# christopherkarani/Wax

Hardware: NVIDIA H100
Metric: queries/sec cosine top-10 @ 10Mx384 fp32 (higher is better)
Workload: dtype f32

## Files before the change

wax_b200/csrc/waxvs_batch.cuh:

```cuda
#pragma once
#include <cuda.h>
#include <cuda_bf16.h>

#include "waxvs_common.cuh"
#include "waxvs_scan.cuh"

namespace waxvs {

constexpr int kBatchM = 128;
constexpr int kBatchN = 128;
constexpr int kBatchKBlock = 32;
constexpr int kBatchKBlockBf16 = 64;
constexpr int kBatchRescore = 256;
constexpr int kBatchRescoreMax = 1024;
constexpr uint32_t kBatchABytes = kBatchM * 128u;
constexpr uint32_t kBatchBBytes = kBatchN * 128u;
constexpr uint32_t kBatchStageBytes = kBatchABytes + kBatchBBytes;
constexpr int kBatchStageSlots = 8;
constexpr uint32_t kBatchScoreStride = kBatchN + 8;
constexpr uint32_t kBatchScoreBytes = kBatchM * kBatchScoreStride * 4u;
constexpr int kBatchMaxStages = 6;
constexpr uint32_t kBatchSmemOptin = 227u * 1024u;
__host__ __device__ constexpr uint32_t batch_smem_bytes(int stages, int heap, uint32_t ares_kb = 0) {
    return ares_kb * kBatchABytes + stages * (ares_kb ? kBatchBBytes : kBatchStageBytes) + kBatchScoreBytes +
// ... 863 lines not shown
        const float *vp[4];
        float d[4];
#pragma unroll
        for (uint32_t r = 0; r < 4; ++r) {
            const uint32_t i = i0 + r * nwarps;
            rows[r] = static_cast<uint32_t>(sk[i < kpp ? i : i0]);
            vp[r] = p.corpus + static_cast<size_t>(rows[r]) * p.dims;
        }
        exact_row_distance_x4<METRIC>(qv, vp, p.dims, s_a2, s_sqrt_a2, lane, d);
        if (lane == 0) {
#pragma unroll
            for (uint32_t r = 0; r < 4; ++r) {
                const uint32_t i = i0 + r * nwarps;
                if (i < kpp) ek[i] = finite_f32(d[r]) ? make_key(d[r], rows[r]) : WAXVS_KEY_NONE;
            }
        }
    }
    __syncthreads();
    block_bitonic_sort(ek, p.rescore);

    if (threadIdx.x == 0) {
        uint32_t n_exact = 0;
        while (n_exact < kpp && ek[n_exact] != WAXVS_KEY_NONE) ++n_exact;
        uint32_t ok = 1;
        float tau_star = -INFINITY, tau_star16 = -INFINITY;
        if (n_exact >= p.k && METRIC == kL2) {
            if constexpr (METRIC == kL2) {
                const float dk = from_orderable_u32(static_cast<uint32_t>(ek[p.k - 1] >> 32));
                l2_proof(s_a2, s_sqrt_a2, dk, tau, __uint_as_float(*p.max_norm_bits), p.dims, p.eps_rel, excluded_any,
                         ok, tau_star, tau_star16);
            }
        } else if (n_exact >= p.k) {
            const float dk = from_orderable_u32(static_cast<uint32_t>(ek[p.k - 1] >> 32));
            const float qn = s_sqrt_a2;
            const float scale = METRIC == kCosine ? qn : qn * __uint_as_float(*p.max_norm_bits);
            const float sk_exact = METRIC == kCosine ? (1.0f - dk) * qn : 1.0f - dk;
            const float acc_slack = static_cast<float>(p.dims) * 0x1p-23f * scale;
            const float ulp_slack = 0x1p-21f * fmaxf(1.0f, fabsf(dk)) * (METRIC == kCosine ? qn : 1.0f);
            const float eps = p.eps_rel * scale * 1.01f + acc_slack + ulp_slack + 1e-30f;
            if (excluded_any && (!(sk_exact > tau + eps) || !finite_f32(eps))) ok = 0;
            const float feps = kTf32Eps * scale * 1.01f + acc_slack + ulp_slack + 1e-30f;
            const float t = sk_exact - feps;
            tau_star = finite_f32(t) ? t - fabsf(t) * 0x1p-20f - 1e-30f : -INFINITY;
            const float feps16 = kBf16Eps * scale * 1.01f + acc_slack + ulp_slack + 1e-30f;
            const float t16 = sk_exact - feps16;
            tau_star16 = finite_f32(t16) ? t16 - fabsf(t16) * 0x1p-20f - 1e-30f : -INFINITY;
        } else if (excluded_any) {
            ok = 0;
        }
        if (METRIC != kL2 && (!(s_a2 >= 0x1p-126f) || !finite_f32(s_a2))) {
            ok = 0;
            tau_star = tau_star16 = -INFINITY;
        }
        p.ok[q] = ok;
        if (p.tau_star) { p.tau_star[q] = tau_star; p.tau_star[p.tau_stride + q] = tau_star16; }
    }
    ScanParams sp{};
    sp.out = p.out + static_cast<size_t>(q) * p.k;
    sp.frame_ids = p.frame_ids; sp.id_base = p.id_base; sp.row_offset = p.row_offset; sp.row_keys = p.row_keys;
    for (uint32_t i = threadIdx.x; i < p.k; i += blockDim.x)
        write_candidate(sp, static_cast<int>(i), i < p.rescore ? ek[i] : WAXVS_KEY_NONE);
}

struct RescoreParams {
    const float *corpus, *query;
    uint32_t dims, k, n_nominees;
    const uint64_t *nominees;
    uint32_t *aux;
    const uint32_t *max_norm_bits;
    float rho_max;
    uint64_t *block_keys;
    uint32_t *ticket;
    uint32_t *work_counter;
    wax_vs_candidate *out;
    uint32_t *ok;
    const uint64_t *frame_ids, *row_keys;
    uint64_t id_base, row_offset;
    uint32_t tail_smem_bytes;
};

template <int METRIC>
__global__ void __launch_bounds__(512, 1) shadow_rescore_kernel(const RescoreParams p) {
    static_assert(METRIC == kCosine || METRIC == kDot, "the shadow route covers cosine and dot");
    extern __shared__ __align__(16) unsigned char rsm[];
    __shared__ float s_a2, s_sqrt_a2;
    const int warp = threadIdx.x >> 5, lane = threadIdx.x & 31, warps = blockDim.x >> 5;
    const int k = static_cast<int>(p.k);
    if (warp == 0) {
        float s0 = 0.f, s1 = 0.f, s2 = 0.f, s3 = 0.f;
        for (uint32_t base = 4u * lane; base < p.dims; base += 128u) {
            const float4 x = __ldg(reinterpret_cast<const float4 *>(p.query + base));
            s0 = __fmaf_rn(x.x, x.x, s0); s1 = __fmaf_rn(x.y, x.y, s1);
            s2 = __fmaf_rn(x.z, x.z, s2); s3 = __fmaf_rn(x.w, x.w, s3);
        }
        const float a2 = warp_butterfly_sum(__fadd_rn(__fadd_rn(s0, s1), __fadd_rn(s2, s3)));
        if (lane == 0) { s_a2 = a2; s_sqrt_a2 = __fsqrt_rn(a2); }
    }
    __shared__ ScanParams sp;
    for (uint32_t i = threadIdx.x; i < sizeof(ScanParams) / 4u; i += blockDim.x) reinterpret_cast<uint32_t *>(&sp)[i] = 0u;
    __syncthreads();
    if (threadIdx.x == 0) {
        sp.k = p.k; sp.block_keys = p.block_keys; sp.ticket = p.ticket; sp.out = p.out;
        sp.frame_ids = p.frame_ids; sp.id_base = p.id_base; sp.row_offset = p.row_offset; sp.row_keys = p.row_keys;
        sp.tail_smem_bytes = p.tail_smem_bytes; sp.work_counter = p.work_counter;
    }
    __syncthreads();

    WarpTopK<1> tk;
    tk.init();
    const uint32_t stride = gridDim.x * warps * 4u;
    for (uint32_t i0 = (blockIdx.x * warps + warp) * 4u; i0 < p.n_nominees; i0 += stride) {
        uint64_t nk[4];
        const float *vp[4];
        float d[4];
#pragma unroll
        for (uint32_t r = 0; r < 4; ++r) {
            nk[r] = i0 + r < p.n_nominees ? p.nominees[i0 + r] : WAXVS_KEY_NONE;
            vp[r] = p.corpus + static_cast<size_t>(nk[r] == WAXVS_KEY_NONE ? 0u : static_cast<uint32_t>(nk[r])) * p.dims;
        }
        exact_row_distance_x4<METRIC>(p.query, vp, p.dims, s_a2, s_sqrt_a2, lane, d);
#pragma unroll
        for (uint32_t r = 0; r < 4; ++r) {
            if (nk[r] == WAXVS_KEY_NONE || !finite_f32(d[r])) continue;
            const uint64_t x = make_key(d[r], static_cast<uint32_t>(nk[r]));
            if (x < tk.thresh) tk.insert(x, lane, k);
        }
    }

    if (!finish_topk_select<1>(sp, tk, rsm)) return;
    __syncthreads();
    if (threadIdx.x != 0) return;
    const wax_vs_candidate kth = p.out[p.k - 1];
    const uint32_t cut = p.aux[0];
    const bool excluded_any = cut != WAXVS_UKEY_NONE;
    const float tau = excluded_any ? -from_orderable_u32(cut) : -INFINITY;
    const float rho_q = __uint_as_float(p.aux[1]);
    uint32_t ok = 1;
    if (kth.valid) {
        const float dk = kth.distance, qn = s_sqrt_a2;
        const float m = METRIC == kCosine ? 1.0f : __uint_as_float(*p.max_norm_bits);
        const float scale = qn * m;
        const float sk_exact = METRIC == kCosine ? (1.0f - dk) * qn : 1.0f - dk;
        const float coding = qn * p.rho_max + rho_q * ((METRIC == kCosine ? 1.0001f : m) + p.rho_max);
        const float acc_slack = static_cast<float>(p.dims) * 0x1p-23f * scale;
        const float ulp_slack = 0x1p-21f * fmaxf(1.0f, fabsf(dk)) * (METRIC == kCosine ? qn : 1.0f);
        const float eps = coding * 1.01f + acc_slack + ulp_slack + 1e-30f;
        if (excluded_any && (!(sk_exact > tau + eps) || !finite_f32(eps))) ok = 0;
    } else if (excluded_any) {
        ok = 0;
    }
    if (!(s_a2 >= 0x1p-126f) || !finite_f32(s_a2)) ok = 0;
    *p.ok = ok;
    p.aux[0] = WAXVS_UKEY_NONE;
    p.aux[2] = cut;
}

template <int METRIC>
__global__ void __launch_bounds__(256) filter_rescore_kernel(const float *corpus, const float *queries, uint32_t dims,
                                                             const uint32_t *cand_count, const uint32_t *cand_rows,
                                                             uint32_t cand_cap, uint64_t *keys) {
    const uint32_t q = blockIdx.y;
    const int lane = threadIdx.x & 31;
    const uint32_t n = min(cand_count[q], cand_cap);
    const uint32_t warps = (gridDim.x * blockDim.x) >> 5;
    uint32_t i = (blockIdx.x * blockDim.x + threadIdx.x) >> 5;
    if (i >= n) return;
// ... 64 lines not shown
```

wax_b200/csrc/waxvs_common.cuh:

```cuda
#pragma once
#include <cuda_runtime.h>
#include <stdint.h>

#define WAXVS_KEY_NONE 0xFFFFFFFFFFFFFFFFull
#define WAXVS_UKEY_NONE 0xFFFFFFFFu
#define WAXVS_FULL_MASK 0xFFFFFFFFu

namespace waxvs {

enum Metric : int { kCosine = 0, kDot = 1, kL2 = 2 };

__device__ __forceinline__ uint32_t orderable_u32(float f) {
    uint32_t u = __float_as_uint(f);
    return u ^ ((u & 0x80000000u) ? 0xFFFFFFFFu : 0x80000000u);
}
__device__ __forceinline__ float from_orderable_u32(uint32_t k) {
    uint32_t u = k ^ ((k & 0x80000000u) ? 0x80000000u : 0xFFFFFFFFu);
    return __uint_as_float(u);
}
__host__ __device__ __forceinline__ bool finite_f32(float f) {
#ifdef __CUDA_ARCH__
    return (__float_as_uint(f) & 0x7F800000u) != 0x7F800000u;
#else
    union { float f; uint32_t u; } x; x.f = f;
// ... 169 lines not shown
                if (pos < 32) {
                    if (lane == pos) key[j] = x;
                    else if (lane > pos) key[j] = up;
                    carry = last;
                    carried = true;
                }
            } else {
                key[j] = (lane == 0) ? carry : up;
                carry = last;
            }
            if (j * 32 + lane >= k) key[j] = WAXVS_KEY_NONE;
        }
        uint64_t t = WAXVS_KEY_NONE;
#pragma unroll
        for (int j = 0; j < E; ++j) {
            const uint64_t cand = shfl_u64(key[j], (k - 1) & 31);
            if (((k - 1) >> 5) == j) t = cand;
        }
        thresh = t;
    }
    __device__ __forceinline__ void merge_sorted(const uint64_t (&other)[E], int lane, int k) {
        if constexpr (E == 1) {
            bitonic_merge_lists<E>(key, thresh, other, lane, k);
        } else {
            TopKRegs<E> a, b;
#pragma unroll
            for (int j = 0; j < E; ++j) { a.key[j] = key[j]; b.key[j] = other[j]; }
            a.thresh = thresh; b.thresh = WAXVS_KEY_NONE;
            a = merge_lists_call<E>(a, b, lane, k);
#pragma unroll
            for (int j = 0; j < E; ++j) key[j] = a.key[j];
            thresh = a.thresh;
        }
    }
};

__device__ __forceinline__ uint32_t smem_u32(const void *p) {
    return static_cast<uint32_t>(__cvta_generic_to_shared(p));
}
__device__ __forceinline__ void mbar_init(uint64_t *bar, uint32_t count) {
    asm volatile("mbarrier.init.shared::cta.b64 [%0], %1;" ::"r"(smem_u32(bar)), "r"(count) : "memory");
}
__device__ __forceinline__ void mbar_fence_init() {
    asm volatile("fence.mbarrier_init.release.cluster;" ::: "memory");
}
__device__ __forceinline__ void mbar_arrive_expect_tx(uint64_t *bar, uint32_t bytes) {
    asm volatile("mbarrier.arrive.expect_tx.shared::cta.b64 _, [%0], %1;" ::"r"(smem_u32(bar)), "r"(bytes)
                 : "memory");
}
__device__ __forceinline__ void mbar_wait_parity(uint64_t *bar, uint32_t parity) {
    const uint32_t addr = smem_u32(bar);
    uint32_t done;
    do {
        asm volatile(
            "{\n\t.reg .pred p;\n\t"
            "mbarrier.try_wait.parity.shared::cta.b64 p, [%1], %2;\n\t"
            "selp.u32 %0, 1, 0, p;\n\t}"
            : "=r"(done)
            : "r"(addr), "r"(parity)
            : "memory");
    } while (!done);
}
__device__ __forceinline__ void bulk_copy_g2s(void *smem_dst, const void *gmem_src, uint32_t bytes,
                                              uint64_t *bar) {
    asm volatile(
        "cp.async.bulk.shared::cluster.global.mbarrier::complete_tx::bytes [%0], [%1], %2, [%3];" ::"r"(
            smem_u32(smem_dst)),
        "l"(gmem_src), "r"(bytes), "r"(smem_u32(bar))
        : "memory");
}
__device__ __forceinline__ void bulk_copy_g2s_hint(void *smem_dst, const void *gmem_src, uint32_t bytes,
                                                   uint64_t *bar, uint64_t policy) {
    asm volatile(
        "cp.async.bulk.shared::cluster.global.mbarrier::complete_tx::bytes.L2::cache_hint [%0], [%1], %2, "
        "[%3], %4;" ::"r"(smem_u32(smem_dst)),
        "l"(gmem_src), "r"(bytes), "r"(smem_u32(bar)), "l"(policy)
        : "memory");
}
__device__ __forceinline__ uint64_t l2_policy_evict_first() {
    uint64_t pol;
    asm volatile("createpolicy.fractional.L2::evict_first.b64 %0, 1.0;" : "=l"(pol));
    return pol;
}
__device__ __forceinline__ uint64_t ld_cg_u64(const uint64_t *p) {
    uint64_t v;
    asm volatile("ld.global.cg.u64 %0, [%1];" : "=l"(v) : "l"(p) : "memory");
    return v;
}

}
```

wax_b200/csrc/waxvs_engine.cu:

```cuda
#include <cuda_runtime.h>

#include <algorithm>
#include <atomic>
#include <cstdarg>
#include <cstdio>
#include <cstring>
#include <limits>
#include <map>
#include <mutex>
#include <new>
#include <shared_mutex>
#include <string>
#include <unordered_map>
#include <chrono>
#include <random>
#include <thread>
#include <unistd.h>
#include <cmath>
#include <vector>

#include "../../include/wax_vs_cuda.h"
#include "waxvs_common.cuh"
#include "waxvs_scan.cuh"
#include "waxvs_select.cuh"
// ... 60 lines not shown
            return fail(WAX_VS_ERR_CUDA, PINNED ? "failed to allocate pinned %s (%zu bytes): %s" : "failed to allocate %s (%zu bytes): %s",
                        what, n * sizeof(T), cudaGetErrorString(cudaGetLastError()));
        cap = n;
        return WAX_VS_OK;
    }
};
template <typename T> using DevBuf = Buf<T, false>;
template <typename T> using PinnedBuf = Buf<T, true>;

struct IdMap {
    std::vector<uint64_t> keys;
    std::vector<uint32_t> vals;
    size_t mask = 0, used = 0;
    static uint64_t mix(uint64_t x) {
        x ^= x >> 30; x *= 0xbf58476d1ce4e5b9ull; x ^= x >> 27; x *= 0x94d049bb133111ebull; x ^= x >> 31;
        return x;
    }
    void reset(size_t expect) {
        size_t cap = 64;
        while (cap < expect * 2 + 16) cap <<= 1;
        keys.assign(cap, 0);
        vals.assign(cap, 0xFFFFFFFFu);
        mask = cap - 1;
        used = 0;
    }
    void prefetch(uint64_t id) const {
        if (vals.empty()) return;
        const size_t i = mix(id) & mask;
        __builtin_prefetch(&keys[i]);
        __builtin_prefetch(&vals[i]);
    }
    uint32_t find(uint64_t id) const {
        if (vals.empty()) return 0xFFFFFFFFu;
        for (size_t i = mix(id) & mask;; i = (i + 1) & mask) {
            if (vals[i] == 0xFFFFFFFFu) return 0xFFFFFFFFu;
            if (keys[i] == id) return vals[i];
        }
    }
    void put(uint64_t id, uint32_t row) {
        if (vals.empty() || (used + 1) * 2 > keys.size()) grow();
        for (size_t i = mix(id) & mask;; i = (i + 1) & mask) {
            if (vals[i] == 0xFFFFFFFFu) { keys[i] = id; vals[i] = row; ++used; return; }
            if (keys[i] == id) { vals[i] = row; return; }
        }
    }
    void grow() {
        std::vector<uint64_t> ok; std::vector<uint32_t> ov;
        ok.swap(keys); ov.swap(vals);
        reset(std::max<size_t>(used * 2, 32));
        for (size_t i = 0; i < ov.size(); ++i) if (ov[i] != 0xFFFFFFFFu) put(ok[i], ov[i]);
    }
};

enum RouteForm : int { kRouteBf16, kRouteInt8, kRouteU4, kRouteForms };

struct Tuning {
    int variant = 0;
    int rows_per_step = 0;
    int stages = 0;
    int warps = 0;
    int grid = 0;
    int l2_hint = 0;
    int ldg_ctas_per_sm = 4;
    int chunk_steps = -1;
    int fused_k_max = 128;
    int batch_tensor = 1;
    int batch_min = 4;
    int time_overlap = 0;
    int batch_pair = 0;
    uint32_t tma_max_dims = 4096;
    int batch_large_k = 1;
    int batch_heap = 0;
    int batch_noinsert = 0;
    int batch_bf16 = 1;
    int batch_ares = 1;
    int batch_rescore = 0;
    int batch_retry = 1;
    int filter_bf16 = 1;
    int filter_cap = 8192;
    int inline_query = 1;
    int host_delivery = 1;
    int tail_select = 1;
    int shard_fused = 1;
    int batch_l2 = 0;
    int single_shadow = 0;
    uint64_t filter_bitset_bytes = 2ull << 30;
    int shadow_scan = 1;
    struct Route { uint64_t min_bytes; int rows_per_step = 0, warps = 0, stages = 0; };
    Route route[kRouteForms] = {
        {512ull << 20},
        {512ull << 20},
        {2048ull << 20},
    };
};

struct SearchCtx {
    cudaStream_t stream = nullptr;
    bool own_stream = false;
    const uint64_t *row_keys = nullptr;
    DevBuf<float> d_queries;
    DevBuf<wax_vs_candidate> d_out;
    PinnedBuf<float> h_queries;
    PinnedBuf<wax_vs_candidate> h_out;
    DevBuf<uint64_t> d_block_keys;
    DevBuf<uint32_t> d_ticket;
    DevBuf<uint32_t> d_dist_keys;
    DevBuf<SelectState> d_select;
    DevBuf<uint64_t> d_sel_keys;
    cudaEvent_t ev0 = nullptr, ev1 = nullptr;
    DevBuf<uint64_t> d_heaps;
    DevBuf<uint32_t> d_ok;
    PinnedBuf<uint32_t> h_ok;
    DevBuf<uint32_t> d_tau;
    DevBuf<__nv_bfloat16> d_queries_bf16;
    DevBuf<float> d_retry_q;
    DevBuf<wax_vs_candidate> d_retry_out;
    DevBuf<uint32_t> d_retry_ok;
    DevBuf<float> d_tau_star;
    PinnedBuf<float> h_tau_star;
    DevBuf<float> d_filter_tau;
    PinnedBuf<float> h_filter_tau;
    DevBuf<uint32_t> d_cand_count;
    DevBuf<uint32_t> d_cand_rows;
    DevBuf<uint64_t> d_cand_keys;
    DevBuf<uint32_t> d_mask;
    DevBuf<uint32_t> d_filter_rows;
    DevBuf<uint64_t> d_filter_spec;
    DevBuf<uint32_t> d_query_filter;
    DevBuf<uint32_t> d_retry_filter;
    DevBuf<uint2> d_gather_span;
    DevBuf<uint64_t> d_gather_keys;
    DevBuf<uint32_t> d_order;
    DevBuf<wax_vs_candidate> d_shard_local;
    DevBuf<unsigned long long> d_group_best;
    DevBuf<uint32_t> d_group_keys;
    DevBuf<uint2> d_group_spans;
    PinnedBuf<uint2> h_group_spans;
    DevBuf<ExpandItem> d_expand_items;
    DevBuf<uint64_t> d_expand[3];
    PinnedBuf<uint64_t> h_expand;
    DevBuf<uint64_t> d_bg_keys;
    PinnedBuf<uint64_t> h_bg_keys;
    DevBuf<uint32_t> d_bg_status;
    PinnedBuf<uint32_t> h_bg_status;
    DevBuf<CoverExpand> d_bg_expand;
    PinnedBuf<CoverExpand> h_bg_expand;
    DevBuf<ScoreItem> d_score_items;
    PinnedBuf<unsigned long long> h_flag;
    unsigned long long host_seq = 0;
    DevBuf<WhereNearItem> d_where_items;
    DevBuf<uint32_t> d_where_counts;
    DevBuf<uint64_t> d_term_ids;
    DevBuf<TermSpan> d_term_spans;
    DevBuf<TermUnit> d_term_units;
    DevBuf<uint32_t> d_term_counts;
    DevBuf<uint32_t> d_term_deny;
    DevBuf<uint32_t> d_proof_count;
    PinnedBuf<uint32_t> h_proof_count;
    uint32_t seen_failed = 0;
    bool last_u4 = false;
    DevBuf<uint32_t> d_u4_aux;
    ~SearchCtx() {
        if (ev0) cudaEventDestroy(ev0);
        if (ev1) cudaEventDestroy(ev1);
        if (own_stream && stream) cudaStreamDestroy(stream);
    }
};

struct wax_vs_engine {
    int device = 0;
    int sm_count = 132;
    size_t smem_optin = 0;
    uint32_t dims = 0;
    uint8_t similarity = 0;

    float *d_corpus = nullptr;
    uint64_t cap_rows = 0, n_rows = 0;

    bool ids_identity = true;
    uint64_t id_base = 0;
    std::vector<uint64_t> ids;
    IdMap map;
    bool map_valid = true;
    bool ids_sorted = true;
    DevBuf<uint64_t> d_ids;
    bool d_ids_dirty = true;
    std::mutex ids_mu;
    bool keys_set = false;
    std::vector<uint64_t> keys;
    DevBuf<uint64_t> d_keys;

    std::shared_mutex rw;
    std::mutex pool_mu;
    std::vector<SearchCtx *> pool;
    std::unordered_map<void *, SearchCtx *> stream_ctx;
    uint64_t pool_allocs = 0, pool_reuses = 0;
    Tuning tune;

    DevBuf<float> d_inv_norm;
    DevBuf<uint32_t> d_max_norm;
    DevBuf<float> d_half_sq;
    uint64_t norms_rows = 0;
    std::mutex norms_mu;
    struct Shadow {
        DevBuf<uint32_t> codes;
        DevBuf<float> scale;
        DevBuf<uint32_t> rho;
        uint64_t rows = 0;
        bool valid = false, unavailable = false;
        bool coarse = false;
        float rho_max = 0.0f, eps_rel = INFINITY;
        void release() { codes.release(); scale.release(); rows = 0; valid = false; }
        void invalidate(uint64_t keep_prefix, bool measured_bound) {
            rows = std::min(rows, keep_prefix);
            if (measured_bound || rows == 0) valid = false;
            if (keep_prefix == 0) coarse = false;
        }
    } shadows[kRouteForms];
    uint32_t u4_demoted = 0, u4_demote_window = 16;
    bool u4_probing = false;
    uint64_t single_route_queries[kRouteForms] = {};
    uint64_t batch_tensor_queries = 0, batch_fallback_queries = 0;
    uint64_t batch_bf16_queries = 0, batch_retry_queries = 0, batch_tf32_queries = 0, batch_filter_bf16_queries = 0;
    uint64_t filter_bitset_passes = 0;
    bool groups_set = false;
    std::vector<uint64_t> groups;
    struct GroupIndex {
        DevBuf<uint32_t> perm, row_group, starts;
        DevBuf<uint64_t> ids;
        uint32_t n_groups = 0;
        bool valid = false;
    } gindex;
    std::mutex group_mu;
    uint64_t group_index_builds = 0;
    bool attrs_set = false;
    std::vector<AttrRow> attrs;
    DevBuf<AttrRow> d_attrs;
    bool attrs_dev_valid = false;
    std::mutex attrs_mu;
    uint64_t attribute_uploads = 0;
    bool locs_set = false;
    std::vector<LocRow> locs;
    DevBuf<LocRow> d_locs;
    bool locs_dev_valid = false;
    uint64_t location_uploads = 0;
    struct TermRef {
        uint64_t off;
        uint32_t n;
    };
    bool terms_set = false;
    std::vector<TermRef> term_refs;
    std::vector<uint64_t> term_pool;
    uint64_t term_garbage = 0;
    struct TermIndex {
        DevBuf<uint64_t> keys, start;
        DevBuf<uint32_t> postings;
        DevBuf<uint64_t> sort_keys, sorted_keys;
        DevBuf<uint32_t> sort_rows, heads, numbering;
        DevBuf<uint8_t> temp;
        uint32_t n_terms = 0;
        uint64_t n_postings = 0;
        bool valid = false;
        void release_scratch() {
            sort_keys.release(); sorted_keys.release(); sort_rows.release(); heads.release(); numbering.release();
            temp.release();
        }
        void release() {
            keys.release(); start.release(); postings.release();
            release_scratch();
            n_terms = 0;
            n_postings = 0;
            valid = false;
        }
    } tindex;
    std::mutex term_mu;
    uint64_t term_index_builds = 0;
    uint64_t grouped_batch_covered_queries = 0, grouped_batch_expanded_groups = 0, grouped_batch_fallback_queries = 0;
    uint64_t grouped_batch_expansion_passes = 0;
    uint64_t shard_grouped_expanded_groups = 0;
    uint32_t bf16_skip_batches = 0;
    uint32_t shadow_scan_skip = 0;
    uint32_t heap_bump = 0, heap_bump_ttl = 0, heap_backoff = 256;
    bool heap_probing = false;
    uint32_t last_heap = 0;
    struct Ingest {
        cudaStream_t stream = nullptr;
        cudaEvent_t ev[2] = {nullptr, nullptr};
        uint8_t *pin[2] = {nullptr, nullptr};
        size_t pin_bytes = 0;
        DevBuf<float> d_stage;
        DevBuf<uint32_t> d_index;
        int threads = 1;
        ~Ingest() {
            for (int i = 0; i < 2; ++i) {
                if (pin[i]) cudaFreeHost(pin[i]);
                if (ev[i]) cudaEventDestroy(ev[i]);
            }
            if (stream) cudaStreamDestroy(stream);
        }
    } ing;
    uint64_t ingest_h2d_bytes = 0, ingest_d2h_bytes = 0;
    std::mutex ingest_mu;
    std::atomic<bool> async_pending{false};
    unsigned long long *debug_trace = nullptr;
// ... 30 lines not shown
    e->tindex.release();
    e->d_attrs.release();
    e->d_locs.release();
    if (SearchCtx *c = e->shard.ctx) {
        c->d_filter_rows.release();
        c->d_mask.release();
        c->d_term_deny.release();
    }
}

static void compact_term_pool(wax_vs_engine *e) {
    if (e->term_garbage * 2 <= e->term_pool.size()) return;
    std::vector<uint64_t> pool;
    pool.reserve(e->term_pool.size() - e->term_garbage);
    for (auto &t : e->term_refs) {
        const uint64_t off = pool.size();
        pool.insert(pool.end(), e->term_pool.begin() + t.off, e->term_pool.begin() + t.off + t.n);
        t.off = t.n ? off : 0;
    }
    e->term_pool.swap(pool);
    e->term_garbage = 0;
}
static void clear_terms(wax_vs_engine *e) {
    e->terms_set = false;
    e->term_refs.clear(); e->term_refs.shrink_to_fit();
    e->term_pool.clear(); e->term_pool.shrink_to_fit();
    e->term_garbage = 0;
    e->tindex.release();
}

static int32_t ctx_new(wax_vs_engine *e, SearchCtx **out, bool with_stream) {
    SearchCtx *c = new (std::nothrow) SearchCtx();
    if (!c) return fail(WAX_VS_ERR_CUDA, "out of host memory");
    auto bail = [&](int32_t rc) { delete c; return rc; };
    if (with_stream) {
        if (cudaStreamCreateWithFlags(&c->stream, cudaStreamNonBlocking) != cudaSuccess)
            return bail(fail(WAX_VS_ERR_CUDA, "cudaStreamCreate failed"));
        c->own_stream = true;
    }
    const size_t block_keys = static_cast<size_t>(std::max(e->sm_count * 8, 2048)) * 128;
    if (cudaMalloc(&c->d_block_keys.p, block_keys * sizeof(uint64_t)) != cudaSuccess ||
        cudaMalloc(&c->d_ticket.p, 4 * sizeof(uint32_t)) != cudaSuccess ||
        cudaMemset(c->d_ticket, 0, 4 * sizeof(uint32_t)) != cudaSuccess ||
        cudaEventCreate(&c->ev0) != cudaSuccess || cudaEventCreate(&c->ev1) != cudaSuccess)
        return bail(fail(WAX_VS_ERR_CUDA, "failed to allocate search scratch: %s",
                         cudaGetErrorString(cudaGetLastError())));
    c->d_block_keys.cap = block_keys;
    c->d_ticket.cap = 4;
    *out = c;
    return WAX_VS_OK;
}

static int32_t ctx_acquire(wax_vs_engine *e, SearchCtx **out) {
    {
        std::lock_guard<std::mutex> g(e->pool_mu);
        if (!e->pool.empty()) {
            *out = e->pool.back();
            e->pool.pop_back();
            ++e->pool_reuses;
            (*out)->row_keys = nullptr;
            return WAX_VS_OK;
        }
        ++e->pool_allocs;
    }
    return ctx_new(e, out, true);
}
static void ctx_release(wax_vs_engine *e, SearchCtx *c) {
    std::lock_guard<std::mutex> g(e->pool_mu);
    e->pool.push_back(c);
}
struct CtxLease {
    wax_vs_engine *e;
    SearchCtx *c = nullptr;
    bool clears_trace = false;
    explicit CtxLease(wax_vs_engine *eng, bool clear_trace = false) : e(eng), clears_trace(clear_trace) {}
    CtxLease(const CtxLease &) = delete;
    CtxLease &operator=(const CtxLease &) = delete;
    ~CtxLease() {
        if (c) ctx_release(e, c);
        if (clears_trace) e->debug_trace = nullptr;
    }
    int32_t acquire() { return ctx_acquire(e, &c); }
};
static int32_t ctx_for_stream(wax_vs_engine *e, void *cuda_stream, SearchCtx **out) {
    std::lock_guard<std::mutex> pg(e->pool_mu);
    auto it = e->stream_ctx.find(cuda_stream);
    if (it != e->stream_ctx.end()) {
        *out = it->second;
        (*out)->row_keys = device_row_keys(e);
        return WAX_VS_OK;
    }
    SearchCtx *c = nullptr;
    int32_t rc = ctx_new(e, &c, false);
    if (rc) return rc;
    c->stream = static_cast<cudaStream_t>(cuda_stream);
    c->row_keys = device_row_keys(e);
    e->stream_ctx[cuda_stream] = c;
    ++e->pool_allocs;
    *out = c;
    return WAX_VS_OK;
}

struct TmaConfig { int C, R, warps, stages; size_t smem; };

constexpr int kUnrolledC[7] = {1, 2, 3, 4, 6, 8, 12};
static int unrolled_index(uint32_t d) {
    for (int i = 0; i < 7; ++i)
        if (d == 128u * kUnrolledC[i]) return i;
    return -1;
}
static size_t tma_smem_budget(const wax_vs_engine *e) { return (e->smem_optin ? e->smem_optin : 232448) - 4096; }
static size_t tma_ring_smem(int warps, int stages, size_t stage_bytes) {
    return static_cast<size_t>(warps) * stages * (stage_bytes + 8 + 4) + static_cast<size_t>(warps) * 1024 + 16;
}

static bool pick_tma_config(const wax_vs_engine *e, TmaConfig *cfg, int mode = 0) {
    const uint32_t d = e->dims;
    if (d % 4u != 0) return false;
    const size_t budget = tma_smem_budget(e);
    const int ci = unrolled_index(d);
    const int C = ci < 0 ? 0 : kUnrolledC[ci];
    if (C == 0 && d < 32) return false;
    if (C == 0 && d > e->tune.tma_max_dims) return false;
    int R, warps_default = 8;
    if (C == 0) {
        int auto_r = d > 256 ? 4 : 8;
        if (d > 640) { auto_r = 8; while (auto_r > 1 && static_cast<size_t>(auto_r) * d * 4 > 32768) auto_r >>= 1; }
        if (d > 3072) auto_r = 1;
        const int want_r = e->tune.rows_per_step;
        R = (want_r == 1 || want_r == 2 || want_r == 4 || want_r == 8) ? want_r : auto_r;
        if (R == 8) warps_default = 16;
        else if (R == 4) warps_default = 12;
    } else if (C == 12) {
        R = e->tune.rows_per_step == 1 || e->tune.rows_per_step == 2 ? e->tune.rows_per_step : 2;
    } else if (C >= 6) {
        R = e->tune.rows_per_step == 2 || e->tune.rows_per_step == 4 ? e->tune.rows_per_step : 2;
    } else {
        R = e->tune.rows_per_step == 4 || e->tune.rows_per_step == 8 ? e->tune.rows_per_step : (C <= 2 ? 8 : 4);
        if (C == 1) warps_default = 16;
        else if (C == 2) warps_default = 12;
        else if (mode == 1 && static_cast<uint64_t>(e->n_rows) * d * 4 < (8ull << 30)) warps_default = 16;
    }
    const int stages = e->tune.stages > 0 ? e->tune.stages : 2;
    const size_t stage_bytes = static_cast<size_t>(R) * d * sizeof(float);
    const size_t query_bytes = C == 0 ? (static_cast<size_t>(d) * 4 + 512 + 32) : 0;
    auto smem_for = [&](int w) { return tma_ring_smem(w, stages, stage_bytes) + query_bytes; };
    int warps = std::max(1, std::min(16, e->tune.warps ? e->tune.warps : warps_default));
    if (!e->tune.warps) while (warps > 2 && smem_for(warps) > budget) --warps;
    if (smem_for(warps) > budget) return false;
    cfg->C = C; cfg->R = R; cfg->warps = warps; cfg->stages = stages; cfg->smem = smem_for(warps);
    return true;
}

template <typename K>
static cudaError_t grant_smem(wax_vs_engine *e, K kernel, size_t bytes) {
    static std::mutex mu;
    static std::map<std::pair<int, const void *>, int> granted;
    std::lock_guard<std::mutex> g(mu);
    int &have = granted[{e->device, reinterpret_cast<const void *>(kernel)}];
    if (have >= static_cast<int>(bytes)) return cudaSuccess;
    cudaError_t err = cudaFuncSetAttribute(kernel, cudaFuncAttributeMaxDynamicSharedMemorySize, static_cast<int>(bytes));
    if (err == cudaSuccess) have = static_cast<int>(bytes);
    return err;
}

template <int C, int R, int M, int E, bool EMIT, bool SHADOW = false, bool INT8 = false, bool U4 = false>
static cudaError_t launch_tma_inst(wax_vs_engine *e, const ScanParams &p, int grid, const TmaConfig &cfg, cudaStream_t s) {
    cudaError_t err = grant_smem(e, scan_tma_kernel<C, R, M, E, EMIT, SHADOW, INT8, U4>, cfg.smem);
    if (err != cudaSuccess) return err;
    scan_tma_kernel<C, R, M, E, EMIT, SHADOW, INT8, U4><<<grid, cfg.warps * 32, cfg.smem, s>>>(p);
    return cudaGetLastError();
}
template <int C, int R>
static cudaError_t launch_tma_cr(wax_vs_engine *e, const ScanParams &p, int grid, const TmaConfig &cfg, int metric, int mode,
                                 cudaStream_t s) {
    switch (metric * 3 + mode) {
        case 0: return launch_tma_inst<C, R, kCosine, 1, false>(e, p, grid, cfg, s);
        case 1: return launch_tma_inst<C, R, kCosine, 4, false>(e, p, grid, cfg, s);
        case 2: return launch_tma_inst<C, R, kCosine, 1, true>(e, p, grid, cfg, s);
        case 3: return launch_tma_inst<C, R, kDot, 1, false>(e, p, grid, cfg, s);
        case 4: return launch_tma_inst<C, R, kDot, 4, false>(e, p, grid, cfg, s);
        case 5: return launch_tma_inst<C, R, kDot, 1, true>(e, p, grid, cfg, s);
        case 6: return launch_tma_inst<C, R, kL2, 1, false>(e, p, grid, cfg, s);
        case 7: return launch_tma_inst<C, R, kL2, 4, false>(e, p, grid, cfg, s);
        default: return launch_tma_inst<C, R, kL2, 1, true>(e, p, grid, cfg, s);
    }
}
static cudaError_t launch_tma(wax_vs_engine *e, const ScanParams &p, int grid, const TmaConfig &cfg, int metric, int mode,
                              cudaStream_t s) {
#define WAXVS_CASE(Cv, Rv) if (cfg.C == Cv && cfg.R == Rv) return launch_tma_cr<Cv, Rv>(e, p, grid, cfg, metric, mode, s)
    WAXVS_CASE(1, 4); WAXVS_CASE(1, 8); WAXVS_CASE(2, 4); WAXVS_CASE(2, 8);
    WAXVS_CASE(3, 4); WAXVS_CASE(3, 8); WAXVS_CASE(4, 4); WAXVS_CASE(4, 8);
    WAXVS_CASE(6, 2); WAXVS_CASE(6, 4); WAXVS_CASE(8, 2); WAXVS_CASE(8, 4);
    WAXVS_CASE(12, 1); WAXVS_CASE(12, 2);
    WAXVS_CASE(0, 1); WAXVS_CASE(0, 2); WAXVS_CASE(0, 4); WAXVS_CASE(0, 8);
#undef WAXVS_CASE
    return cudaErrorInvalidValue;
}
template <RouteForm F, int C, int R>
static cudaError_t launch_route_cr(wax_vs_engine *e, const ScanParams &p, int grid, const TmaConfig &cfg, int metric,
                                   cudaStream_t s) {
    if constexpr (F == kRouteU4) {
        return launch_tma_inst<C, R, kDot, 4, false, true, false, true>(e, p, grid, cfg, s);
    } else {
        return metric == kCosine ? launch_tma_inst<C, R, kCosine, 4, false, true, F == kRouteInt8>(e, p, grid, cfg, s)
                                 : launch_tma_inst<C, R, kDot, 4, false, true, F == kRouteInt8>(e, p, grid, cfg, s);
    }
}
#define WAXVS_CASE(Cv, Rv) \
    if (cfg.C == Cv && cfg.R == Rv) return p ? launch_route_cr<F, Cv, Rv>(e, *p, grid, cfg, metric, s) : cudaSuccess
static cudaError_t launch_shadow_scan(wax_vs_engine *e, const ScanParams *p, int grid, const TmaConfig &cfg, int metric,
                                      cudaStream_t s) {
    constexpr RouteForm F = kRouteBf16;
    WAXVS_CASE(1, 8); WAXVS_CASE(1, 16); WAXVS_CASE(2, 8); WAXVS_CASE(2, 16);
    WAXVS_CASE(3, 4); WAXVS_CASE(3, 8); WAXVS_CASE(3, 16); WAXVS_CASE(4, 4); WAXVS_CASE(4, 8);
    WAXVS_CASE(6, 2); WAXVS_CASE(6, 4); WAXVS_CASE(8, 2); WAXVS_CASE(8, 4); WAXVS_CASE(12, 2); WAXVS_CASE(12, 4);
    return cudaErrorInvalidValue;
}
static cudaError_t launch_int8_scan(wax_vs_engine *e, const ScanParams *p, int grid, const TmaConfig &cfg, int metric,
                                   cudaStream_t s) {
    constexpr RouteForm F = kRouteInt8;
    WAXVS_CASE(1, 8); WAXVS_CASE(1, 16); WAXVS_CASE(2, 8); WAXVS_CASE(2, 16);
    WAXVS_CASE(3, 4); WAXVS_CASE(3, 8); WAXVS_CASE(3, 16); WAXVS_CASE(4, 4); WAXVS_CASE(4, 8);
    WAXVS_CASE(6, 4); WAXVS_CASE(6, 8); WAXVS_CASE(8, 4); WAXVS_CASE(12, 4);
    return cudaErrorInvalidValue;
}
static cudaError_t launch_u4_scan(wax_vs_engine *e, const ScanParams *p, int grid, const TmaConfig &cfg, int metric,
                                  cudaStream_t s) {
    constexpr RouteForm F = kRouteU4;
    WAXVS_CASE(1, 8); WAXVS_CASE(1, 16); WAXVS_CASE(2, 8); WAXVS_CASE(2, 16); WAXVS_CASE(3, 8); WAXVS_CASE(3, 16);
    WAXVS_CASE(4, 4); WAXVS_CASE(4, 8); WAXVS_CASE(6, 4); WAXVS_CASE(6, 8); WAXVS_CASE(8, 4); WAXVS_CASE(12, 4);
    return cudaErrorInvalidValue;
}
#undef WAXVS_CASE

struct RouteFormSpec {
    const char *name;
    uint32_t bits;
    bool scaled;
    cudaError_t (*launch)(wax_vs_engine *, const ScanParams *, int, const TmaConfig &, int, cudaStream_t);
    int default_r[7];
    int warps, stages;
    bool keep_warps;
    bool grid_rescore;
    uint32_t tail_bytes;
    float max_eps_rel;
};
constexpr RouteFormSpec kRouteSpec[kRouteForms] = {
    {"bf16", 16, false, launch_shadow_scan, {8, 8, 4, 4, 2, 2, 2}, 16, 3, false, false, 2, kBf16Eps},
    {"int8", 8, true, launch_int8_scan, {8, 8, 8, 4, 4, 4, 4}, 16, 3, false, false, 1, kBf16Eps},
    {"4-bit", 4, true, launch_u4_scan, {16, 16, 16, 8, 8, 4, 4}, 16, 3, true, true, 2, std::numeric_limits<float>::max()},
};
// ... 54 lines not shown
        }
    }
}

static int32_t stage_queries(wax_vs_engine *e, SearchCtx *c, const float *queries, uint32_t n, cudaStream_t stream,
                             const uint32_t *order = nullptr) {
    const size_t qfloats = static_cast<size_t>(n) * e->dims;
    int32_t rc = c->d_queries.ensure(qfloats, "query buffer");
    if (!rc) rc = c->h_queries.ensure(qfloats, "query staging");
    if (rc) return rc;
    if (order) {
        for (uint32_t j = 0; j < n; ++j)
            memcpy(c->h_queries + static_cast<size_t>(j) * e->dims, queries + static_cast<size_t>(order[j]) * e->dims,
                   e->dims * sizeof(float));
    } else {
        memcpy(c->h_queries, queries, qfloats * sizeof(float));
    }
    CUDA_TRY(cudaMemcpyAsync(c->d_queries, c->h_queries, qfloats * sizeof(float), cudaMemcpyHostToDevice, stream));
    return WAX_VS_OK;
}

struct HostDelivery {
    const float *h_query;
    wax_vs_candidate *host_out;
    unsigned long long *host_flag;
    unsigned long long seq;
    bool delivered = false;
};

static int32_t enqueue_select(wax_vs_engine *e, SearchCtx *c, const uint32_t *keys, uint32_t n, uint32_t k,
                              const ScanParams &p, cudaStream_t stream, uint64_t *launches) {
    int32_t rc = c->d_select.ensure(1, "selection state");
    if (!rc) rc = c->d_sel_keys.ensure(16384, "selected keys");
    if (rc) return rc;
    const int sgrid = std::max(1, std::min<int>(e->sm_count * 4, static_cast<int>((n + 511) / 512)));
    select_init_kernel<<<1, 256, 0, stream>>>(c->d_select, k);
    for (int pass = 0; pass < kSelectPasses; ++pass) {
        select_hist_kernel<<<sgrid, 512, 0, stream>>>(keys, n, c->d_select, pass);
        select_scan_kernel<<<1, 1024, 0, stream>>>(c->d_select, pass);
    }
    select_compact_kernel<<<sgrid, 512, 0, stream>>>(keys, n, c->d_select, c->d_sel_keys, 16384);
    uint32_t pow2 = 64;
    while (pow2 < k) pow2 <<= 1;
    CUDA_TRY(grant_smem(e, select_sort_kernel, pow2 * sizeof(uint64_t)));
    select_sort_kernel<<<1, 1024, pow2 * sizeof(uint64_t), stream>>>(c->d_select, c->d_sel_keys, pow2, p);
    CUDA_TRY(cudaGetLastError());
    *launches += 3 + 2 * kSelectPasses;
    return WAX_VS_OK;
}

static int tma_grid(const wax_vs_engine *e, const SearchCtx *c, const TmaConfig &cfg, ScanParams &p) {
    p.stages = static_cast<uint32_t>(cfg.stages);
    const uint64_t steps = (e->n_rows + cfg.R - 1) / cfg.R;
    const int max_grid = e->tune.grid > 0 ? e->tune.grid : e->sm_count;
    int grid = static_cast<int>(std::min<uint64_t>(max_grid, (steps + cfg.warps - 1) / cfg.warps));
    grid = std::max(std::min(grid, static_cast<int>(c->d_block_keys.cap / 128)), 1);
    if (e->tune.chunk_steps < 0)
        p.chunk_steps = static_cast<uint32_t>(std::max<uint64_t>(1, std::min<uint64_t>(8, steps / (static_cast<uint64_t>(grid) * cfg.warps * 2))));
    return grid;
}

static bool batch_bf16_wanted(const wax_vs_engine *e);
static int32_t ensure_shadow(wax_vs_engine *e, cudaStream_t stream);
static int32_t ensure_coded_shadow(wax_vs_engine *e, RouteForm f, cudaStream_t stream, bool keep_coarse);
static int32_t ensure_route_shadow(wax_vs_engine *e, RouteForm f, cudaStream_t stream, bool keep_coarse = false) {
    return f == kRouteBf16 ? ensure_shadow(e, stream) : ensure_coded_shadow(e, f, stream, keep_coarse);
}

constexpr uint32_t kShadowNominees = 128;
constexpr uint32_t kShadowRescore = 256;
constexpr uint32_t kShadowSkipQueries = 16;
static bool shadow_route_applies(const wax_vs_engine *e) {
    return e->tune.shadow_scan && (e->similarity == WAX_VS_COSINE || e->similarity == WAX_VS_DOT) && !e->debug_trace &&
           e->tune.batch_bf16 != 0 && e->dims % kBatchKBlockBf16 == 0 &&
           e->n_rows * e->dims * sizeof(float) >= e->tune.route[kRouteBf16].min_bytes;
}
static int32_t select_route_form(wax_vs_engine *e, cudaStream_t stream, bool demoted, bool *use, RouteForm *form,
                                 TmaConfig *cfg) {
    *use = false;
    for (const RouteForm f : {kRouteU4, kRouteInt8, kRouteBf16}) {
        if ((f == kRouteU4 && demoted) || e->n_rows * e->dims * sizeof(float) < e->tune.route[f].min_bytes ||
            !pick_route_config(e, f, cfg))
            continue;
        if (const int32_t rc = ensure_route_shadow(e, f, stream)) return rc;
        if (e->shadows[f].valid && e->shadows[f].eps_rel <= kRouteSpec[f].max_eps_rel) {
            *use = true;
            *form = f;
            return WAX_VS_OK;
        }
    }
    return WAX_VS_OK;
}

static int32_t enqueue_shadow_nominations(wax_vs_engine *e, SearchCtx *c, const ScanParams &p, const TmaConfig &cfg,
                                          cudaStream_t stream, uint64_t *launches, uint32_t *shape, RouteForm f) {
    const RouteFormSpec &fs = kRouteSpec[f];
    const wax_vs_engine::Shadow &sh = e->shadows[f];
    int32_t rc;
    if (fs.grid_rescore && !c->d_u4_aux) {
        if ((rc = c->d_u4_aux.ensure(3, "4-bit route state"))) return rc;
        CUDA_TRY(cudaMemsetAsync(c->d_u4_aux, 0xFF, 3 * sizeof(uint32_t), stream));
    }
    const size_t cta_keys = static_cast<size_t>(std::max(e->tune.grid, e->sm_count)) * kU4CtaNominees;
    if ((rc = c->d_heaps.ensure(std::max(static_cast<size_t>(kShadowNominees) * kNomineeStride, fs.grid_rescore ? cta_keys : 0), "nominee keys")) ||
        (rc = c->d_ok.ensure(1, "proof flags")) || (!p.query && (rc = c->d_queries.ensure(e->dims, "query buffer"))))
        return rc;

    ScanParams sp = p;
    sp.corpus = reinterpret_cast<const float *>(sh.codes.p);
    sp.row_scale = fs.scaled ? sh.scale.p : nullptr;
    sp.u4_aux = fs.grid_rescore ? c->d_u4_aux.p : nullptr;
    sp.k = kShadowNominees;
    sp.out = nullptr; sp.host_out = nullptr; sp.host_flag = nullptr;
    sp.nominees = c->d_heaps;
    sp.query_store = p.query ? nullptr : c->d_queries.p;
    sp.tail_select = e->tune.tail_select ? 1u : 0u;
    sp.tail_smem_bytes = static_cast<uint32_t>(static_cast<size_t>(cfg.warps) * cfg.stages * cfg.R * e->dims * fs.tail_bytes);
    const int grid = tma_grid(e, c, cfg, sp);
    CUDA_TRY(fs.launch(e, &sp, grid, cfg, e->similarity, stream));

    if (fs.grid_rescore) {
        RescoreParams rp{};
        rp.corpus = e->d_corpus; rp.query = p.query ? p.query : c->d_queries.p;
        rp.dims = e->dims; rp.k = p.k; rp.n_nominees = static_cast<uint32_t>(grid) * kU4CtaNominees;
        rp.nominees = c->d_heaps; rp.aux = c->d_u4_aux; rp.max_norm_bits = e->d_max_norm; rp.rho_max = sh.rho_max;
        rp.block_keys = c->d_block_keys; rp.ticket = c->d_ticket; rp.work_counter = sp.work_counter; rp.out = p.out; rp.ok = c->d_ok;
        rp.frame_ids = p.frame_ids; rp.id_base = p.id_base; rp.row_offset = p.row_offset; rp.row_keys = p.row_keys;
        rp.tail_smem_bytes = static_cast<uint32_t>(grid) * p.k * sizeof(uint64_t);
        if (rp.tail_smem_bytes > 48u * 1024u) rp.tail_smem_bytes = 0;
        const auto kernel = e->similarity == WAX_VS_COSINE ? shadow_rescore_kernel<kCosine> : shadow_rescore_kernel<kDot>;
        kernel<<<grid, 512, rp.tail_smem_bytes, stream>>>(rp);
        CUDA_TRY(cudaGetLastError());
    } else {
        FinishParams fp{};
        fp.corpus = e->d_corpus; fp.queries = p.query ? p.query : c->d_queries.p;
        fp.n_rows = p.n_rows; fp.dims = e->dims; fp.n_queries = 1; fp.groups = 1; fp.slices = 1;
        fp.kprime = kShadowNominees; fp.k = p.k; fp.metric = e->similarity;
        fp.heaps = c->d_heaps; fp.max_norm_bits = e->d_max_norm;
        fp.out = p.out; fp.ok = c->d_ok;
        fp.frame_ids = p.frame_ids; fp.id_base = p.id_base; fp.row_offset = p.row_offset; fp.row_keys = p.row_keys;
        fp.pow2_all = 512; fp.rescore = kShadowRescore; fp.eps_rel = sh.eps_rel;
        const size_t fsmem = static_cast<size_t>(fp.pow2_all + fp.rescore) * sizeof(uint64_t);
        const auto kernel = e->similarity == WAX_VS_COSINE ? batch_finish_kernel<kCosine> : batch_finish_kernel<kDot>;
        CUDA_TRY(grant_smem(e, kernel, fsmem));
        kernel<<<1, 512, fsmem, stream>>>(fp);
        CUDA_TRY(cudaGetLastError());
    }
    *launches += 2;
    if (shape) {
        const uint32_t s[7] = {static_cast<uint32_t>(cfg.C), static_cast<uint32_t>(cfg.R), static_cast<uint32_t>(cfg.warps),
                               static_cast<uint32_t>(cfg.stages), static_cast<uint32_t>(grid), sp.chunk_steps, sp.tail_select};
        std::copy(s, s + 7, shape);
    }
    return WAX_VS_OK;
}

static int32_t enqueue_shadow_route(wax_vs_engine *e, SearchCtx *c, ScanParams &p, cudaStream_t stream, uint64_t *launches) {
    if (!shadow_route_applies(e)) return WAX_VS_OK;
    int32_t rc;
    if (!c->h_proof_count) {
        if ((rc = c->d_proof_count.ensure(2, "proof counts")) || (rc = c->h_proof_count.ensure(2, "proof count mirror"))) return rc;
        CUDA_TRY(cudaMemsetAsync(c->d_proof_count, 0, 2 * sizeof(uint32_t), stream));
        c->h_proof_count[0] = c->h_proof_count[1] = 0;
        c->seen_failed = 0;
    }
    bool demoted;
    {
        std::lock_guard<std::mutex> pg(e->pool_mu);
        const uint32_t failed = *static_cast<volatile uint32_t *>(c->h_proof_count + 1);
        if (failed != c->seen_failed) {
            c->seen_failed = failed;
            if (c->last_u4) {
                if (e->u4_probing) e->u4_demote_window = std::min(e->u4_demote_window * 2, 1u << 20);
                e->u4_demoted = e->u4_demote_window;
            } else {
                e->shadow_scan_skip = kShadowSkipQueries;
            }
        } else if (c->last_u4 && e->u4_probing) {
            e->u4_demote_window = 16;
        }
        if (c->last_u4) e->u4_probing = false;
        c->last_u4 = false;
        if (e->shadow_scan_skip > 0) { --e->shadow_scan_skip; return WAX_VS_OK; }
        demoted = e->u4_demoted > 0;
        if (demoted && --e->u4_demoted == 0) e->u4_probing = true;
    }
    bool use = false;
    RouteForm form = kRouteBf16;
    TmaConfig cfg{};
    if ((rc = select_route_form(e, stream, demoted, &use, &form, &cfg)) || !use) return rc;
    if ((rc = enqueue_shadow_nominations(e, c, p, cfg, stream, launches, nullptr, form))) return rc;
    c->last_u4 = form == kRouteU4;
    {
        std::lock_guard<std::mutex> pg(e->pool_mu);
        ++e->single_route_queries[form];
    }
    p.proof_ok = c->d_ok;
    p.proof_count = c->d_proof_count;
    p.proof_count_host = c->h_proof_count;
    return WAX_VS_OK;
}

static ScanParams scan_params(const wax_vs_engine *e, SearchCtx *c, const float *d_query, uint32_t k_eff, uint64_t row_offset,
                              wax_vs_candidate *d_out, const uint64_t *d_ids, const uint32_t *d_mask) {
    ScanParams p{};
    p.corpus = e->d_corpus; p.query = d_query;
    p.n_rows = static_cast<uint32_t>(e->n_rows); p.dims = e->dims; p.k = k_eff;
    p.block_keys = c->d_block_keys; p.ticket = c->d_ticket; p.out = d_out;
    p.frame_ids = d_ids; p.id_base = e->id_base; p.row_offset = row_offset; p.row_keys = c->row_keys;
    p.use_l2_hint = e->tune.l2_hint ? 1u : 0u;
    p.chunk_steps = e->tune.chunk_steps > 0 ? static_cast<uint32_t>(e->tune.chunk_steps) : 0u;
    p.work_counter = c->d_ticket + 1;
    p.mask = d_mask;
    p.trace = e->debug_trace;
    return p;
}

static int32_t place_host_query(wax_vs_engine *e, SearchCtx *c, ScanParams &p, const float *h_query, bool inline_ok,
                                cudaStream_t stream) {
    if (inline_ok && e->tune.inline_query != 0 && e->dims <= static_cast<uint32_t>(kInlineQueryFloats)) {
        memcpy(p.query_inline, h_query, e->dims * sizeof(float));
        p.query = nullptr;
        return WAX_VS_OK;
    }
    int32_t rc = stage_queries(e, c, h_query, 1, stream);
    if (rc) return rc;
    p.query = c->d_queries;
    return WAX_VS_OK;
}

static int32_t enqueue_exchange(const ShardParams &sp, const wax_vs_candidate *local, uint32_t k, cudaStream_t stream,
                                uint64_t *launches) {
    shard_exchange_kernel<<<1, 256, 0, stream>>>(sp, local, k);
    CUDA_TRY(cudaGetLastError());
    ++*launches;
    return WAX_VS_OK;
}

static int32_t enqueue_search(wax_vs_engine *e, SearchCtx *c, const float *d_query, uint32_t k_eff,
                              uint64_t row_offset, wax_vs_candidate *d_out, const uint64_t *d_ids,
                              cudaStream_t stream, uint64_t *launches, const uint32_t *d_mask = nullptr,
                              const ShardParams *shard = nullptr, const HostDelivery *host = nullptr,
                              bool keys_only = false, bool shadow_route = false) {
    wax_vs_candidate *d_merged = nullptr;
    if (shard) {
        if (k_eff > static_cast<uint32_t>(kShardKCap))
            return fail(WAX_VS_ERR_UNSUPPORTED, "sharded search supports top_k <= %d (got %u)", kShardKCap, k_eff);
        int32_t rc = c->d_shard_local.ensure(kShardKCap, "shard candidates");
        if (rc) return rc;
        d_merged = d_out;
        d_out = c->d_shard_local;
    }
    auto exchange_standalone = [&]() -> int32_t {
        ShardParams sp = *shard;
        sp.final_out = d_merged;
        return enqueue_exchange(sp, d_out, k_eff, stream, launches);
    };
    if (e->n_rows == 0) {
        CUDA_TRY(cudaMemsetAsync(d_out, 0, static_cast<size_t>(k_eff) * sizeof(wax_vs_candidate), stream));
        return shard ? exchange_standalone() : WAX_VS_OK;
    }
    ScanParams p = scan_params(e, c, d_query, k_eff, row_offset, d_out, d_ids, d_mask);
    const bool emit = keys_only || k_eff > static_cast<uint32_t>(e->tune.fused_k_max);
    const int mode = emit ? 2 : (k_eff <= 32 ? 0 : 1);
    if (emit) {
        int32_t rc = c->d_dist_keys.ensure(static_cast<size_t>(e->n_rows), "distance keys");
        if (rc) return rc;
        p.dist_keys = c->d_dist_keys;
    }

    TmaConfig cfg{};
    bool use_tma = (e->tune.variant != 2) && pick_tma_config(e, &cfg, mode);
    if (e->tune.variant == 1 && !use_tma)
        return fail(WAX_VS_ERR_UNSUPPORTED, "TMA-staged kernel does not support dims=%u", e->dims);
    if (host && host->h_query) {
        int32_t rc = place_host_query(e, c, p, host->h_query, use_tma && !emit, stream);
        if (rc) return rc;
    }
    if (host && host->host_out && !emit && !shard) {
        p.host_out = host->host_out; p.host_flag = host->host_flag; p.host_seq = host->seq;
        const_cast<HostDelivery *>(host)->delivered = true;
    }
    if (use_tma && !emit && e->tune.tail_select) {
        p.tail_select = 1u;
        p.tail_smem_bytes = static_cast<uint32_t>(static_cast<size_t>(cfg.warps) * cfg.stages * cfg.R * e->dims * sizeof(float));
    }
    bool fused_exchange = false;
    if (shard && !emit) {
        const size_t list_bytes = p.tail_select ? p.tail_smem_bytes
                                                : static_cast<size_t>(use_tma ? cfg.warps : 8) * 32 * (mode == 0 ? 1 : 4) * sizeof(uint64_t);
        fused_exchange = e->tune.shard_fused != 0 && static_cast<size_t>(shard->world) * k_eff * sizeof(uint32_t) <= list_bytes;
        if (fused_exchange) { p.shard = *shard; p.shard.final_out = d_merged; }
    }
    if (shadow_route && !shard && mode == 0 && use_tma && cfg.C > 0) {
        int32_t rc = enqueue_shadow_route(e, c, p, stream, launches);
        if (rc) return rc;
    }
    int grid;
    const int grid_cap = static_cast<int>(c->d_block_keys.cap / 128);
    if (use_tma) {
        grid = tma_grid(e, c, cfg, p);
        CUDA_TRY(launch_tma(e, p, grid, cfg, e->similarity, mode, stream));
    } else {
        const int max_grid = e->tune.grid > 0 ? e->tune.grid : e->sm_count * e->tune.ldg_ctas_per_sm;
        grid = static_cast<int>(std::min<uint64_t>(max_grid, (e->n_rows + 7) / 8));
        grid = std::max(std::min(grid, grid_cap), 1);
        CUDA_TRY(launch_ldg(p, grid, e->similarity, mode, stream));
    }
    ++*launches;

    if (emit && !keys_only) {
        int32_t rc = enqueue_select(e, c, c->d_dist_keys, static_cast<uint32_t>(e->n_rows), k_eff, p, stream, launches);
        if (rc) return rc;
    }
    if (shard && !fused_exchange) return exchange_standalone();
    return WAX_VS_OK;
}

static PFN_cuTensorMapEncodeTiled_v12000 tensor_map_encoder() {
    static PFN_cuTensorMapEncodeTiled_v12000 fn = nullptr;
    static std::once_flag once;
    std::call_once(once, [] {
        void *ptr = nullptr;
        cudaDriverEntryPointQueryResult q;
        if (cudaGetDriverEntryPoint("cuTensorMapEncodeTiled", &ptr, cudaEnableDefault, &q) == cudaSuccess &&
            q == cudaDriverEntryPointSuccess)
            fn = reinterpret_cast<PFN_cuTensorMapEncodeTiled_v12000>(ptr);
    });
    return fn;
}

static int32_t make_tensor_map(CUtensorMap *map, const void *base, uint64_t rows, uint32_t dims, uint32_t box_rows,
                               bool bf16 = false) {
    auto enc = tensor_map_encoder();
    if (!enc) return fail(WAX_VS_ERR_CUDA, "cuTensorMapEncodeTiled is not available from this driver");
    const size_t esize = bf16 ? sizeof(__nv_bfloat16) : sizeof(float);
    const cuuint64_t gdim[2] = {dims, rows};
    const cuuint64_t gstride[1] = {static_cast<cuuint64_t>(dims) * esize};
    const cuuint32_t box[2] = {static_cast<cuuint32_t>(bf16 ? kBatchKBlockBf16 : kBatchKBlock), box_rows};
    const cuuint32_t estr[2] = {1, 1};
    const CUresult r = enc(map, bf16 ? CU_TENSOR_MAP_DATA_TYPE_BFLOAT16 : CU_TENSOR_MAP_DATA_TYPE_FLOAT32, 2,
                           const_cast<void *>(base), gdim, gstride, box, estr, CU_TENSOR_MAP_INTERLEAVE_NONE,
                           CU_TENSOR_MAP_SWIZZLE_128B, CU_TENSOR_MAP_L2_PROMOTION_L2_256B, CU_TENSOR_MAP_FLOAT_OOB_FILL_NONE);
    if (r != CUDA_SUCCESS) return fail(WAX_VS_ERR_CUDA, "cuTensorMapEncodeTiled failed (CUresult %d)", static_cast<int>(r));
    return WAX_VS_OK;
}

static bool batch_bf16_wanted(const wax_vs_engine *e);
static bool batch_tensor_eligible(const wax_vs_engine *e, uint32_t n_queries, uint32_t k_eff) {
    const uint32_t min_batch = (e->tune.single_shadow && batch_bf16_wanted(e)) ? 1u : static_cast<uint32_t>(std::max(e->tune.batch_min, 1));
    return e->tune.batch_tensor && n_queries >= min_batch &&
           (e->similarity == WAX_VS_COSINE || e->similarity == WAX_VS_DOT || (e->similarity == WAX_VS_L2 && e->tune.batch_l2)) &&
           e->dims % kBatchKBlock == 0 &&
           e->dims <= 8192 &&
           k_eff >= 1 && e->n_rows >= 1 &&
           (k_eff <= 128 || (k_eff <= static_cast<uint32_t>(kBatchRescoreMax) && e->tune.batch_large_k &&
                             n_queries >= static_cast<uint32_t>(std::max(e->tune.batch_min, 4)) &&
                             e->n_rows >= 64ull * k_eff));
}

static int32_t ensure_norms_locked(wax_vs_engine *e, cudaStream_t stream) {
    const bool l2 = e->similarity == WAX_VS_L2;
    if (e->norms_rows == e->n_rows && e->d_inv_norm && (!l2 || e->d_half_sq)) return WAX_VS_OK;
    if (static_cast<size_t>(e->n_rows) > e->d_inv_norm.cap || !e->d_inv_norm ||
        (l2 && (static_cast<size_t>(e->n_rows) > e->d_half_sq.cap || !e->d_half_sq))) {
        e->norms_rows = 0;
        const size_t want = static_cast<size_t>(std::max<uint64_t>(e->cap_rows, std::max<uint64_t>(e->n_rows, 1)));
        int32_t rc = e->d_inv_norm.ensure(want, "row norms");
        if (!rc && l2) rc = e->d_half_sq.ensure(want, "row half squared norms");
        if (rc) return rc;
    }
    if (!e->d_max_norm) {
        int32_t rc = e->d_max_norm.ensure(1, "max row norm");
        if (rc) return rc;
        e->norms_rows = 0;
    }
    if (e->norms_rows > e->n_rows) e->norms_rows = 0;
    if (e->norms_rows == 0) CUDA_TRY(cudaMemsetAsync(e->d_max_norm, 0, sizeof(uint32_t), stream));
// ... 717 lines not shown
        parallel_memcpy(static_cast<char *>(h_dst) + off, pin[i & 1], len, g.threads);
    }
    CUDA_TRY(cudaStreamSynchronize(g.stream));
    return WAX_VS_OK;
}

static int32_t add_batch_rows(wax_vs_engine *e, const uint64_t *frame_ids, const float *rows, uint64_t n,
                              uint32_t vector_len, const uint64_t *first_key, uint64_t *out_appended) {
    if (!e) return fail(WAX_VS_ERR_NULL, "engine is NULL");
    if (out_appended) *out_appended = 0;
    if (n == 0) return WAX_VS_OK;
    if (!frame_ids || !rows) return fail(WAX_VS_ERR_NULL, "NULL argument");
    if (vector_len != e->dims)
        return fail(WAX_VS_ERR_DIMENSION, "vector dimension mismatch: expected %u, got %u", e->dims, vector_len);
    IngestTrace tr("add_batch");
    std::unique_lock<std::shared_mutex> w(e->rw);
    if (first_key && e->n_rows > 0) {
        const uint64_t last = e->keys_set ? e->keys.back() : e->n_rows - 1;
        if (*first_key <= last)
            return fail(WAX_VS_ERR_ARGUMENT, "first key %llu is not above the last row key %llu",
                        static_cast<unsigned long long>(*first_key), static_cast<unsigned long long>(last));
    }
    DeviceGuard g(e->device);
    drain_device_path(e);
    tr.mark("lock+drain");
    int32_t rc = grow_for(e, e->n_rows + n);
    if (rc) return rc;
    if (first_key && (rc = materialize_row_keys(e))) return rc;
    tr.mark("grow");
    materialize_ids(e);
    tr.mark("ids");

    std::vector<uint32_t> target(n);
    const uint64_t n0 = e->n_rows;
    bool pure_append = true;
    bool increasing = e->ids_sorted && (e->ids.empty() || frame_ids[0] > e->ids.back());
    for (uint64_t i = 1; i < n && increasing; ++i) increasing = frame_ids[i] > frame_ids[i - 1];
    if (increasing) {
        e->ids.insert(e->ids.end(), frame_ids, frame_ids + n);
        if (e->groups_set) e->groups.insert(e->groups.end(), frame_ids, frame_ids + n);
        if (e->attrs_set) e->attrs.resize(e->attrs.size() + n, AttrRow{0, 0});
        if (e->locs_set) e->locs.resize(e->locs.size() + n, LocRow{kNoLocation, 0});
        if (e->terms_set) e->term_refs.resize(e->term_refs.size() + n, wax_vs_engine::TermRef{0, 0});
        for (uint64_t i = 0; i < n; ++i) target[i] = static_cast<uint32_t>(n0 + i);
        e->n_rows += n;
        e->map_valid = false;
    } else {
        for (uint64_t i = 0; i < n; ++i) {
            if (!e->ids_sorted && i + 8 < n) e->map.prefetch(frame_ids[i + 8]);
            uint32_t row = find_row(e, frame_ids[i]);
            if (row == 0xFFFFFFFFu) {
                row = static_cast<uint32_t>(e->n_rows);
                if (e->ids_sorted && !e->ids.empty() && frame_ids[i] < e->ids.back()) {
                    e->ids_sorted = false;
                    e->map_valid = false;
                    ensure_map(e);
                }
                e->ids.push_back(frame_ids[i]);
                if (e->groups_set) e->groups.push_back(frame_ids[i]);
                if (e->attrs_set) e->attrs.push_back(AttrRow{0, 0});
                if (e->locs_set) e->locs.push_back(LocRow{kNoLocation, 0});
                if (e->terms_set) e->term_refs.push_back(wax_vs_engine::TermRef{0, 0});
                if (!e->ids_sorted) e->map.put(frame_ids[i], row);
                else e->map_valid = false;
                ++e->n_rows;
            }
            target[i] = row;
            if (row != n0 + i) pure_append = false;
        }
    }
    e->d_ids_dirty = true;
    if (out_appended) *out_appended = e->n_rows - n0;
    if (e->keys_set) {
        const uint64_t base = first_key ? *first_key : (n0 ? e->keys.back() + 1 : 0);
        for (uint64_t r = n0; r < e->n_rows; ++r) e->keys.push_back(base + (r - n0));
        if ((rc = upload_row_keys(e, n0))) return rc;
    }
    const size_t row_bytes = static_cast<size_t>(e->dims) * sizeof(float);
    tr.mark("resolve targets");
    if (pure_append) {
        invalidate_row_caches(e, n0);
        rc = upload_bytes(e, e->d_corpus + n0 * e->dims, rows, n * row_bytes);
        tr.mark("upload");
        return rc;
    }
    invalidate_row_caches(e, 0);
    {
        std::unordered_map<uint32_t, uint64_t> last;
        last.reserve(n * 2);
        for (uint64_t i = 0; i < n; ++i) last[target[i]] = i;
        for (uint64_t i = 0; i < n; ++i) if (last[target[i]] != i) target[i] = 0xFFFFFFFFu;
    }
    auto &ig = e->ing;
    if ((rc = ingest_init(e))) return rc;
    const uint64_t slab_rows = std::max<uint64_t>(1, std::min<uint64_t>(n, (size_t(256) << 20) / row_bytes));
    if ((rc = ig.d_stage.ensure(static_cast<size_t>(slab_rows) * e->dims, "upsert staging"))) return rc;
    if ((rc = ig.d_index.ensure(static_cast<size_t>(slab_rows), "upsert targets"))) return rc;
    for (uint64_t done = 0; done < n; done += slab_rows) {
        const uint64_t m = std::min(slab_rows, n - done);
        if ((rc = upload_bytes(e, ig.d_stage, rows + done * e->dims, m * row_bytes))) return rc;
        CUDA_TRY(cudaMemcpyAsync(ig.d_index, target.data() + done, m * sizeof(uint32_t), cudaMemcpyHostToDevice, ig.stream));
        scatter_rows_kernel<<<static_cast<unsigned>(m), 128, 0, ig.stream>>>(e->d_corpus, ig.d_stage, ig.d_index, m, e->dims);
        CUDA_TRY(cudaGetLastError());
        CUDA_TRY(cudaStreamSynchronize(ig.stream));
    }
    return WAX_VS_OK;
}

int32_t wax_vs_add_batch(wax_vs_engine *e, const uint64_t *frame_ids, const float *rows, uint64_t n,
                         uint32_t vector_len) {
    return add_batch_rows(e, frame_ids, rows, n, vector_len, nullptr, nullptr);
}

int32_t wax_vs_add_batch_keyed(wax_vs_engine *e, const uint64_t *frame_ids, const float *rows, uint64_t n,
                               uint32_t vector_len, uint64_t first_key, uint64_t *out_appended) {
    return add_batch_rows(e, frame_ids, rows, n, vector_len, &first_key, out_appended);
}

int32_t wax_vs_add(wax_vs_engine *e, uint64_t frame_id, const float *vector, uint32_t vector_len) {
    return wax_vs_add_batch(e, &frame_id, vector, 1, vector_len);
}

int32_t wax_vs_contains(wax_vs_engine *e, const uint64_t *frame_ids, uint64_t n, uint8_t *out) {
    if (!e) return fail(WAX_VS_ERR_NULL, "engine is NULL");
    if (n == 0) return WAX_VS_OK;
    if (!frame_ids || !out) return fail(WAX_VS_ERR_NULL, "NULL argument");
    std::shared_lock<std::shared_mutex> r(e->rw);
    std::lock_guard<std::mutex> g(e->ids_mu);
    for (uint64_t i = 0; i < n; ++i) out[i] = row_of(e, frame_ids[i]) != 0xFFFFFFFFu;
    return WAX_VS_OK;
}

int32_t wax_vs_remove_batch(wax_vs_engine *e, const uint64_t *frame_ids, uint64_t n, uint64_t *out_removed) {
    if (!e) return fail(WAX_VS_ERR_NULL, "engine is NULL");
    if (out_removed) *out_removed = 0;
    if (n == 0) return WAX_VS_OK;
    if (!frame_ids) return fail(WAX_VS_ERR_NULL, "frame_ids is NULL");
    IngestTrace tr("remove_batch");
    std::unique_lock<std::shared_mutex> w(e->rw);
    if (e->n_rows == 0) return WAX_VS_OK;
    std::vector<uint32_t> gone;
    gone.reserve(n);
    for (uint64_t i = 0; i < n; ++i) {
        const uint32_t r = row_of(e, frame_ids[i]);
        if (r != 0xFFFFFFFFu) gone.push_back(r);
    }
    if (gone.empty()) return WAX_VS_OK;
    std::sort(gone.begin(), gone.end());
    gone.erase(std::unique(gone.begin(), gone.end()), gone.end());
    DeviceGuard g(e->device);
    drain_device_path(e);
    materialize_ids(e);
    const uint64_t old_n = e->n_rows, first = gone.front(), new_n = old_n - gone.size();
    std::vector<uint32_t> src;
    src.reserve(static_cast<size_t>(new_n - first));
    {
        size_t gi = 0;
        for (uint64_t r = first; r < old_n; ++r) {
            if (gi < gone.size() && gone[gi] == r) { ++gi; continue; }
            src.push_back(static_cast<uint32_t>(r));
        }
    }
    tr.mark("resolve rows + sources");
    int32_t rc = ingest_init(e);
    if (rc) return rc;
    auto &ig = e->ing;
    const size_t row_bytes = static_cast<size_t>(e->dims) * sizeof(float);
    const uint64_t moving = src.size();
    if (moving) {
        const uint64_t slab_rows = std::max<uint64_t>(1, std::min<uint64_t>(moving, (size_t(256) << 20) / row_bytes));
        if ((rc = ig.d_stage.ensure(static_cast<size_t>(slab_rows) * e->dims, "compaction bounce buffer"))) return rc;
        if ((rc = ig.d_index.ensure(static_cast<size_t>(slab_rows), "compaction sources"))) return rc;
        if ((rc = ingest_staging(e, slab_rows * sizeof(uint32_t)))) return rc;
        for (uint64_t done = 0; done < moving; done += slab_rows) {
            const uint64_t m = std::min(slab_rows, moving - done);
            const bool contiguous = src[done + m - 1] - src[done] == m - 1;
            float *dst = e->d_corpus + (first + done) * e->dims;
            if (contiguous) {
                CUDA_TRY(cudaMemcpyAsync(ig.d_stage, e->d_corpus + static_cast<uint64_t>(src[done]) * e->dims, m * row_bytes,
                                         cudaMemcpyDeviceToDevice, ig.stream));
            } else {
                CUDA_TRY(cudaMemcpyAsync(ig.d_index, src.data() + done, m * sizeof(uint32_t), cudaMemcpyHostToDevice, ig.stream));
                const unsigned grid = static_cast<unsigned>(std::min<uint64_t>(m, static_cast<uint64_t>(e->sm_count) * 32));
                gather_rows_kernel<<<grid, 128, 0, ig.stream>>>(ig.d_stage, e->d_corpus, ig.d_index, m, e->dims);
                CUDA_TRY(cudaGetLastError());
            }
            CUDA_TRY(cudaMemcpyAsync(dst, ig.d_stage, m * row_bytes, cudaMemcpyDeviceToDevice, ig.stream));
            CUDA_TRY(cudaStreamSynchronize(ig.stream));
        }
    }
    tr.mark("compact matrix");
    if (e->terms_set)
        for (const uint32_t r : gone) e->term_garbage += e->term_refs[r].n;
    for (uint64_t j = 0; j < moving; ++j) {
        e->ids[first + j] = e->ids[src[j]];
        if (e->groups_set) e->groups[first + j] = e->groups[src[j]];
        if (e->attrs_set) e->attrs[first + j] = e->attrs[src[j]];
        if (e->locs_set) e->locs[first + j] = e->locs[src[j]];
        if (e->terms_set) e->term_refs[first + j] = e->term_refs[src[j]];
        if (e->keys_set) e->keys[first + j] = e->keys[src[j]];
    }
    e->ids.resize(new_n);
    if (e->keys_set) e->keys.resize(new_n);
    if (e->groups_set) e->groups.resize(new_n);
    if (e->attrs_set) e->attrs.resize(new_n);
    if (e->locs_set) e->locs.resize(new_n);
    if (e->terms_set) {
        e->term_refs.resize(new_n);
        compact_term_pool(e);
    }
    e->n_rows = new_n;
    e->map_valid = false;
    e->d_ids_dirty = true;
    invalidate_row_caches(e, first);
    if ((rc = upload_row_keys(e, first))) return rc;
    tr.mark("compact ids");
    if (out_removed) *out_removed = gone.size();
    return WAX_VS_OK;
}

int32_t wax_vs_remove(wax_vs_engine *e, uint64_t frame_id) {
    return wax_vs_remove_batch(e, &frame_id, 1, nullptr);
}

static int32_t enqueue_filter_level(wax_vs_engine *e, SearchCtx *c, const float *d_queries, const float *d_tau,
                                    uint32_t n_queries, uint32_t k_eff, uint64_t row_offset, wax_vs_candidate *d_out,
                                    uint32_t *d_ok, const uint64_t *d_ids, cudaStream_t stream, uint64_t *launches,
                                    bool bf16 = false, const RowFilter &rf = RowFilter{}) {
    int32_t rc = ensure_norms(e, stream);
    if (rc) return rc;
    uint32_t cap = 64;
    while ((cap < static_cast<uint32_t>(std::max(e->tune.filter_cap, 64)) || cap < k_eff) && cap < 16384u) cap <<= 1;
    if ((rc = c->d_cand_count.ensure(static_cast<size_t>(n_queries), "filter counts"))) return rc;
    if ((rc = c->d_cand_rows.ensure(static_cast<size_t>(n_queries) * cap, "filter candidates"))) return rc;
    if ((rc = c->d_cand_keys.ensure(static_cast<size_t>(n_queries) * cap, "filter keys"))) return rc;
    CUDA_TRY(cudaMemsetAsync(c->d_cand_count, 0, static_cast<size_t>(n_queries) * sizeof(uint32_t), stream));
    auto prepare = [&](const NominateChunk &ch, BatchParams &bp) -> int32_t {
        bp.tau_fixed = d_tau + ch.q0;
        bp.cand_count = c->d_cand_count + ch.q0;
        bp.cand_rows = c->d_cand_rows + static_cast<size_t>(ch.q0) * cap;
        bp.cand_cap = cap;
        return WAX_VS_OK;
    };
    auto finish = [&](const NominateChunk &ch) -> int32_t {
        const uint32_t *count = c->d_cand_count + ch.q0;
        uint64_t *keys = c->d_cand_keys + static_cast<size_t>(ch.q0) * cap;
        const auto rescore = e->similarity == WAX_VS_COSINE ? filter_rescore_kernel<kCosine>
                             : e->similarity == WAX_VS_DOT  ? filter_rescore_kernel<kDot>
                                                            : filter_rescore_kernel<kL2>;
        rescore<<<dim3(32, ch.nq), 256, 0, stream>>>(e->d_corpus, ch.queries, e->dims, count,
                                                     c->d_cand_rows + static_cast<size_t>(ch.q0) * cap, cap, keys);
        CUDA_TRY(cudaGetLastError());
        FilterSelectParams sp{};
        sp.cand_count = count; sp.keys = keys; sp.cand_cap = cap; sp.k = k_eff;
        sp.out = d_out + static_cast<size_t>(ch.q0) * k_eff; sp.ok = d_ok + ch.q0;
        sp.frame_ids = d_ids; sp.id_base = e->id_base; sp.row_offset = row_offset; sp.row_keys = c->row_keys;
        const size_t ssmem = static_cast<size_t>(cap) * sizeof(uint64_t);
        CUDA_TRY(grant_smem(e, filter_select_kernel, ssmem));
        filter_select_kernel<<<ch.nq, 1024, ssmem, stream>>>(sp);
        CUDA_TRY(cudaGetLastError());
        *launches += 2;
        return WAX_VS_OK;
    };
    return enqueue_nominate_pass(e, c, d_queries, n_queries, bf16, true, false, false, static_cast<uint32_t>(e->sm_count),
                                 rf, stream, launches, [](uint32_t, uint32_t) { return 16u; }, prepare, finish);
}

static int32_t enqueue_scans(wax_vs_engine *e, SearchCtx *c, const float *d_queries, uint32_t n, const uint32_t *qs,
                             uint32_t k_eff, uint64_t row_offset, wax_vs_candidate *d_out, const uint64_t *d_ids,
                             cudaStream_t stream, uint64_t *launches, const RowFilter &rf, bool sync_on_error,
                             bool shadow_route = false) {
    for (uint32_t i = 0; i < n; ++i) {
        const uint32_t qi = qs ? qs[i] : i;
        const int32_t rc = enqueue_search(e, c, d_queries + static_cast<size_t>(qi) * e->dims, k_eff, row_offset,
                                          d_out + static_cast<size_t>(qi) * k_eff, d_ids, stream, launches, rf.mask(qi),
                                          nullptr, nullptr, false, shadow_route);
        if (rc) {
            if (sync_on_error) cudaStreamSynchronize(stream);
            return rc;
        }
    }
    return WAX_VS_OK;
}

static int32_t run_queries_on_device(wax_vs_engine *e, SearchCtx *c, const float *d_queries, uint32_t n_queries,
                                     uint32_t k_eff, uint64_t row_offset, wax_vs_candidate *d_out, const uint64_t *d_ids,
                                     uint64_t *launches, const RowFilter &rf = RowFilter{}) {
    int32_t rc = WAX_VS_OK;
    bool tensor_path = batch_tensor_eligible(e, n_queries, k_eff), allow_bf16 = true;
    if (tensor_path) {
        std::lock_guard<std::mutex> pg(e->pool_mu);
        if (e->bf16_skip_batches > 0) { --e->bf16_skip_batches; allow_bf16 = false; }
    }
    if (tensor_path && !allow_bf16 && n_queries < static_cast<uint32_t>(std::max(e->tune.batch_min, 1))) tensor_path = false;
    if (!tensor_path)
        return enqueue_scans(e, c, d_queries, n_queries, nullptr, k_eff, row_offset, d_out, d_ids, c->stream, launches, rf, true,
                             true);
    if ((rc = c->d_ok.ensure(static_cast<size_t>(n_queries), "proof flags"))) return rc;
    if ((rc = c->h_ok.ensure(static_cast<size_t>(n_queries), "proof flag staging"))) return rc;
    if ((rc = c->d_tau_star.ensure(static_cast<size_t>(n_queries) * 2, "filter thresholds"))) return rc;
    if ((rc = c->h_tau_star.ensure(static_cast<size_t>(n_queries) * 2, "filter threshold staging"))) return rc;
// ... 276 lines not shown
        ++*launches;
    }
    return WAX_VS_OK;
}
static int32_t stage_filter_rows(wax_vs_engine *e, SearchCtx *c, const std::vector<uint32_t> &rows, size_t reserve,
                                 int32_t mode, cudaStream_t stream, uint64_t *launches) {
    int32_t rc;
    if ((rc = c->d_filter_rows.ensure(std::max<size_t>(reserve, 1), "filter rows"))) return rc;
    if (!rows.empty())
        CUDA_TRY(cudaMemcpyAsync(c->d_filter_rows, rows.data(), rows.size() * sizeof(uint32_t), cudaMemcpyHostToDevice, stream));
    if (mode < 0) return WAX_VS_OK;
    return build_filter_bits(e, c, {0, rows.size(), 0, static_cast<uint64_t>(mode)}, 1, stream, launches);
}

struct ShardHandle {
    uint32_t magic, version;
    int32_t pid, device;
    uint64_t nonce;
    uint64_t ptr;
    int32_t rank, world;
    cudaIpcMemHandle_t ipc;
    uint8_t pad[WAX_VS_SHARD_HANDLE_BYTES - 40 - sizeof(cudaIpcMemHandle_t)];
};
static_assert(sizeof(ShardHandle) == WAX_VS_SHARD_HANDLE_BYTES, "handle blob size");
static uint64_t process_nonce() {
    static const uint64_t n = [] { std::random_device rd; return (static_cast<uint64_t>(rd()) << 32) ^ rd() ^ 0x9E3779B97F4A7C15ull; }();
    return n;
}

static void shard_teardown(wax_vs_engine *e, bool free_own) {
    auto &sh = e->shard;
    if (!sh.open) return;
    cudaDeviceSynchronize();
    for (int r = 0; r < sh.world; ++r) {
        if (r != sh.rank && sh.ipc[r] && sh.box[r]) cudaIpcCloseMemHandle(sh.box[r]);
        sh.ipc[r] = false;
        if (r != sh.rank) sh.box[r] = nullptr;
    }
    sh.connected = false;
    cudaGetLastError();
    if (!free_own) return;
    if (sh.box[sh.rank]) cudaFree(sh.box[sh.rank]);
    sh.box[sh.rank] = nullptr;
    delete sh.ctx;
    sh.ctx = nullptr;
    cudaGetLastError();
    sh.open = false;
    sh.seq = 0;
}

int32_t wax_vs_shard_open(wax_vs_engine *e, int32_t rank, int32_t world, uint64_t row_offset, uint8_t *out_handle) {
    if (!e || !out_handle) return fail(WAX_VS_ERR_NULL, "NULL argument");
    if (world < 1 || world > kShardMaxRanks || rank < 0 || rank >= world)
        return fail(WAX_VS_ERR_ARGUMENT, "rank %d of %d: world must be 1..%d", rank, world, kShardMaxRanks);
    std::unique_lock<std::shared_mutex> w(e->rw);
    DeviceGuard g(e->device);
    if (!g.ok) return g.error();
    drain_device_path(e);
    shard_teardown(e, true);
    auto &sh = e->shard;
    ShardMailbox *box = nullptr;
    CUDA_TRY(cudaMalloc(&box, sizeof(ShardMailbox)));
    int32_t rc = sh.d_final.ensure(kShardKCap, "shard result");
    if (!rc) rc = sh.h_final.ensure(kShardKCap, "shard result delivery");
    if (!rc) rc = sh.h_flag.ensure(1, "shard completion flag");
    if (rc) { cudaFree(box); return rc; }
    cudaError_t err = cudaMemset(box, 0, sizeof(ShardMailbox));
    if (err == cudaSuccess) err = cudaDeviceSynchronize();
    ShardHandle h{};
    if (err == cudaSuccess) err = cudaIpcGetMemHandle(&h.ipc, box);
    if (err != cudaSuccess) {
        cudaFree(box);
        return fail(WAX_VS_ERR_CUDA, "failed to create the shard mailbox: %s", cudaGetErrorString(err));
    }
    *sh.h_flag = 0;
    if ((rc = ctx_new(e, &sh.ctx, true))) { cudaFree(box); return rc; }
    sh.rank = rank; sh.world = world; sh.row_offset = row_offset;
    sh.box[rank] = box;
    sh.open = true; sh.connected = (world == 1);
    sh.seq = 0;
    h.magic = 0x48535857u; h.version = 1; h.pid = static_cast<int32_t>(getpid()); h.device = e->device;
    h.nonce = process_nonce(); h.ptr = reinterpret_cast<uint64_t>(box); h.rank = rank; h.world = world;
    memcpy(out_handle, &h, sizeof h);
    return WAX_VS_OK;
}

int32_t wax_vs_shard_connect(wax_vs_engine *e, const uint8_t *handles, int32_t n_handles) {
    if (!e || !handles) return fail(WAX_VS_ERR_NULL, "NULL argument");
    std::unique_lock<std::shared_mutex> w(e->rw);
    auto &sh = e->shard;
    if (!sh.open) return fail(WAX_VS_ERR_ARGUMENT, "wax_vs_shard_open has not been called");
    if (n_handles != sh.world) return fail(WAX_VS_ERR_ARGUMENT, "expected %d handles, got %d", sh.world, n_handles);
    DeviceGuard g(e->device);
    if (!g.ok) return g.error();
    for (int r = 0; r < sh.world; ++r) {
        ShardHandle h;
        memcpy(&h, handles + static_cast<size_t>(r) * sizeof h, sizeof h);
        if (h.magic != 0x48535857u || h.version != 1 || h.rank != r || h.world != sh.world)
            return fail(WAX_VS_ERR_ARGUMENT, "handle %d is not rank %d of %d", r, r, sh.world);
        if (r == sh.rank) continue;
        if (h.pid == static_cast<int32_t>(getpid()) && h.nonce == process_nonce()) {
            if (h.device != e->device) {
                int can = 0;
                CUDA_TRY(cudaDeviceCanAccessPeer(&can, e->device, h.device));
                if (!can) return fail(WAX_VS_ERR_UNSUPPORTED, "device %d cannot access device %d (no P2P path)", e->device, h.device);
                cudaError_t pe = cudaDeviceEnablePeerAccess(h.device, 0);
                if (pe != cudaSuccess && pe != cudaErrorPeerAccessAlreadyEnabled)
                    return fail(WAX_VS_ERR_CUDA, "cudaDeviceEnablePeerAccess(%d) failed: %s", h.device, cudaGetErrorString(pe));
                cudaGetLastError();
            }
            sh.box[r] = reinterpret_cast<ShardMailbox *>(h.ptr);
            sh.ipc[r] = false;
        } else {
            void *ptr = nullptr;
            cudaError_t ie = cudaIpcOpenMemHandle(&ptr, h.ipc, cudaIpcMemLazyEnablePeerAccess);
            if (ie != cudaSuccess) {
                cudaGetLastError();
                return fail(WAX_VS_ERR_UNSUPPORTED, "cudaIpcOpenMemHandle for rank %d failed: %s (no P2P/IPC path between the ranks)",
                            r, cudaGetErrorString(ie));
            }
            sh.box[r] = static_cast<ShardMailbox *>(ptr);
            sh.ipc[r] = true;
        }
    }
    sh.connected = true;
    return WAX_VS_OK;
}

int32_t wax_vs_shard_close(wax_vs_engine *e) {
    if (!e) return fail(WAX_VS_ERR_NULL, "engine is NULL");
    std::unique_lock<std::shared_mutex> w(e->rw);
    DeviceGuard g(e->device);
    shard_teardown(e, false);
    return WAX_VS_OK;
}

static ShardParams shard_params_next(wax_vs_engine *e) {
    auto &sh = e->shard;
    ShardParams sp{};
    for (int r = 0; r < sh.world; ++r) sp.box[r] = sh.box[r];
    sp.rank = static_cast<uint32_t>(sh.rank); sp.world = static_cast<uint32_t>(sh.world);
    sp.seq = ++sh.seq;
    sp.timeout_ns = sh.timeout_ns;
    return sp;
}

int32_t wax_vs_shard_search_device(wax_vs_engine *e, const float *d_query, int64_t top_k, wax_vs_candidate *d_candidates,
                                   void *cuda_stream) {
    if (!e || !d_query || !d_candidates) return fail(WAX_VS_ERR_NULL, "NULL argument");
    std::shared_lock<std::shared_mutex> r(e->rw);
    if (!e->shard.connected) return fail(WAX_VS_ERR_ARGUMENT, "the shard group is not connected (wax_vs_shard_open / _connect)");
    DeviceGuard g(e->device);
    if (!g.ok) return g.error();
    const uint32_t k_eff = clamp_topk(top_k);
    if (k_eff > static_cast<uint32_t>(kShardKCap))
        return fail(WAX_VS_ERR_UNSUPPORTED, "sharded search supports top_k <= %d (got %u)", kShardKCap, k_eff);
    SearchCtx *c = nullptr;
    int32_t rc = ctx_for_stream(e, cuda_stream, &c);
    if (rc) return rc;
    e->async_pending.store(true);
    const uint64_t *d_ids = nullptr;
    if ((rc = sync_device_ids(e, &d_ids))) return rc;
    std::lock_guard<std::mutex> sg(e->shard.mu);
    ShardParams sp = shard_params_next(e);
    uint64_t launches = 0;
    return enqueue_search(e, c, d_query, k_eff, e->shard.row_offset, d_candidates, d_ids,
                          static_cast<cudaStream_t>(cuda_stream), &launches, nullptr, &sp);
}

static int32_t shard_wait_host(wax_vs_engine *e, unsigned long long seq) {
    int32_t rc = wait_host_flag(e->shard.ctx->stream, e->shard.h_flag, seq, e->shard.timeout_ns);
    if (rc == 1)
        return fail(WAX_VS_ERR_CUDA, "shard exchange timed out: a peer rank did not deliver its candidates for query #%llu", seq);
    return rc;
}

struct Clause;
static int32_t shard_search_host(wax_vs_engine *e, const float *query, uint32_t query_len, int64_t top_k, bool filtered,
                                 const uint64_t *frame_ids, uint64_t n_ids, int32_t mode, const Clause *where,
                                 uint64_t *out_ids, float *out_scores, uint32_t out_cap, uint32_t *out_n);

int32_t wax_vs_shard_search(wax_vs_engine *e, const float *query, uint32_t query_len, int64_t top_k, uint64_t *out_ids,
                            float *out_scores, uint32_t out_cap, uint32_t *out_n) {
    if (!e || !out_n) return fail(WAX_VS_ERR_NULL, "NULL argument");
    return shard_search_host(e, query, query_len, top_k, false, nullptr, 0, 0, nullptr, out_ids, out_scores, out_cap, out_n);
}

int32_t wax_vs_debug_time_shard_search(wax_vs_engine *e, uint32_t n_queries, int64_t top_k, uint64_t seed, uint32_t warmup,
                                       uint32_t iters, float *out_ms_total, uint64_t *out_launches) {
    if (!e || !out_ms_total) return fail(WAX_VS_ERR_NULL, "NULL argument");
    if (n_queries == 0) n_queries = 1;
    std::shared_lock<std::shared_mutex> r(e->rw);
    if (!e->shard.connected) return fail(WAX_VS_ERR_ARGUMENT, "the shard group is not connected (wax_vs_shard_open / _connect)");
    DeviceGuard g(e->device);
    auto &sh = e->shard;
    std::lock_guard<std::mutex> sg(sh.mu);
    SearchCtx *c = sh.ctx;
    c->row_keys = device_row_keys(e);
    const uint32_t k_eff = clamp_topk(top_k);
    int32_t rc;
    if ((rc = c->d_queries.ensure(static_cast<size_t>(n_queries) * e->dims, "query buffer"))) return rc;
    synth_fill_kernel<<<(n_queries + 255) / 256, 256, 0, c->stream>>>(c->d_queries, n_queries, e->dims, seed, 0, 1);
    CUDA_TRY(cudaGetLastError());
    const uint64_t *d_ids = nullptr;
    if ((rc = sync_device_ids(e, &d_ids))) return rc;
    uint64_t launches = 0;
    for (uint32_t it = 0; it < warmup + iters; ++it) {
        if (it == warmup) { launches = 0; CUDA_TRY(cudaEventRecord(c->ev0, c->stream)); }
        ShardParams sp = shard_params_next(e);
        rc = enqueue_search(e, c, c->d_queries + static_cast<size_t>(it % n_queries) * e->dims, k_eff, sh.row_offset,
                            sh.d_final, d_ids, c->stream, &launches, nullptr, &sp);
        if (rc) { cudaStreamSynchronize(c->stream); return rc; }
    }
    CUDA_TRY(cudaEventRecord(c->ev1, c->stream));
    CUDA_TRY(cudaStreamSynchronize(c->stream));
    CUDA_TRY(cudaEventElapsedTime(out_ms_total, c->ev0, c->ev1));
    if (out_launches) *out_launches = launches;
    return WAX_VS_OK;
}

int32_t wax_vs_merge_candidates_device(wax_vs_engine *e, const wax_vs_candidate *d_gathered, uint32_t world,
                                       uint32_t n_queries, uint32_t k, uint32_t k_out, wax_vs_candidate *d_out,
                                       void *cuda_stream) {
    if (!e || !d_gathered || !d_out) return fail(WAX_VS_ERR_NULL, "NULL argument");
    if (world == 0 || world > 1024u || k == 0 || k_out == 0 || k_out > k)
        return fail(WAX_VS_ERR_ARGUMENT, "merge: world %u, k %u, k_out %u", world, k, k_out);
    if (n_queries == 0) return WAX_VS_OK;
    DeviceGuard g(e->device);
    if (!g.ok) return g.error();
    merge_gathered_kernel<<<n_queries, 128, 0, static_cast<cudaStream_t>(cuda_stream)>>>(d_gathered, world, n_queries, k, k_out, d_out);
    CUDA_TRY(cudaGetLastError());
    return WAX_VS_OK;
}

static int32_t ensure_locations(wax_vs_engine *e, SearchCtx *c) {
    if (e->locs_dev_valid) return WAX_VS_OK;
    const size_t n = static_cast<size_t>(e->n_rows);
    int32_t rc;
    if ((rc = e->d_locs.ensure(std::max<size_t>(n, 1), "row locations"))) return rc;
    const std::vector<LocRow> none(e->locs_set ? 0 : n, LocRow{kNoLocation, 0});
    CUDA_TRY(cudaMemcpyAsync(e->d_locs, e->locs_set ? e->locs.data() : none.data(), n * sizeof(LocRow),
                             cudaMemcpyHostToDevice, c->stream));
    CUDA_TRY(cudaStreamSynchronize(c->stream));
    e->locs_dev_valid = true;
    std::lock_guard<std::mutex> pg(e->pool_mu);
    ++e->location_uploads;
    return WAX_VS_OK;
}
static int32_t ensure_attributes(wax_vs_engine *e, SearchCtx *c, bool locations = false) {
    std::lock_guard<std::mutex> lk(e->attrs_mu);
    int32_t rc;
    if (locations && (rc = ensure_locations(e, c))) return rc;
    if (e->attrs_dev_valid) return WAX_VS_OK;
    const size_t n = static_cast<size_t>(e->n_rows);
    if ((rc = e->d_attrs.ensure(std::max<size_t>(n, 1), "row attributes"))) return rc;
    if (e->attrs_set) CUDA_TRY(cudaMemcpyAsync(e->d_attrs, e->attrs.data(), n * sizeof(AttrRow), cudaMemcpyHostToDevice, c->stream));
    else CUDA_TRY(cudaMemsetAsync(e->d_attrs, 0, n * sizeof(AttrRow), c->stream));
    CUDA_TRY(cudaStreamSynchronize(c->stream));
    e->attrs_dev_valid = true;
    std::lock_guard<std::mutex> pg(e->pool_mu);
    ++e->attribute_uploads;
    return WAX_VS_OK;
}

static int32_t ensure_term_index(wax_vs_engine *e, SearchCtx *c) {
    std::lock_guard<std::mutex> lk(e->term_mu);
    auto &ti = e->tindex;
    if (ti.valid) return WAX_VS_OK;
    uint64_t n_pairs = 0;
    if (e->terms_set)
        for (const auto &t : e->term_refs) n_pairs += t.n;
    if (n_pairs > static_cast<uint64_t>(INT32_MAX))
        return fail(WAX_VS_ERR_CAPACITY, "term index of %llu (term, row) pairs: at most %d are supported",
                    static_cast<unsigned long long>(n_pairs), INT32_MAX);
    const uint32_t P = static_cast<uint32_t>(n_pairs);
    cudaStream_t s = c->stream;
    int32_t rc;
    uint32_t n_terms = 0;
    if ((rc = ti.postings.ensure(std::max<uint32_t>(P, 1), "term postings"))) return rc;
    if (P) {
        std::vector<uint64_t> h_keys(P);
        std::vector<uint32_t> h_rows(P);
        for (uint64_t r = 0, at = 0; r < e->n_rows; ++r) {
            const auto &t = e->term_refs[r];
            for (uint32_t j = 0; j < t.n; ++j, ++at) {
                h_keys[at] = e->term_pool[t.off + j];
                h_rows[at] = static_cast<uint32_t>(r);
            }
        }
        auto &keys_in = ti.sort_keys, &keys_out = ti.sorted_keys;
        auto &rows_in = ti.sort_rows, &heads = ti.heads, &incl = ti.numbering;
        auto &temp = ti.temp;
        size_t sort_bytes = 0, scan_bytes = 0;
        CUDA_TRY(cub::DeviceRadixSort::SortPairs(nullptr, sort_bytes, keys_in.p, keys_out.p, rows_in.p, ti.postings.p,
// ... 850 lines not shown
    }
    std::vector<uint32_t> written(static_cast<size_t>((e->n_rows + 31) / 32), 0u);
    std::vector<uint64_t> list;
    uint64_t assigned = 0;
    for (uint64_t i = 0; i < n; ++i) {
        const uint32_t row = row_of(e, frame_ids[i]);
        if (row == 0xFFFFFFFFu) continue;
        list.assign(terms + term_offsets[i], terms + term_offsets[i + 1]);
        std::sort(list.begin(), list.end());
        list.erase(std::unique(list.begin(), list.end()), list.end());
        auto &ref = e->term_refs[row];
        e->term_garbage += ref.n;
        ref = wax_vs_engine::TermRef{list.empty() ? 0 : e->term_pool.size(), static_cast<uint32_t>(list.size())};
        e->term_pool.insert(e->term_pool.end(), list.begin(), list.end());
        const uint32_t wd = row >> 5, b = 1u << (row & 31u);
        if (!(written[wd] & b)) { written[wd] |= b; ++assigned; }
    }
    compact_term_pool(e);
    e->tindex.release();
    if (out_assigned) *out_assigned = assigned;
    return WAX_VS_OK;
}

static int32_t term_clauses(const wax_vs_where_near *wheres, uint32_t n_wheres, const uint32_t *query_where,
                            uint32_t n_queries, const uint64_t *where_term_offsets, const uint64_t *where_terms,
                            std::vector<Clause> &clauses, std::vector<uint32_t> &qw) {
    int32_t rc;
    if ((rc = check_term_offsets(where_term_offsets, n_wheres, where_terms, kMaxWhereTerms, "where_term_offsets"))) return rc;
    if ((rc = near_clauses(wheres, n_wheres, clauses))) return rc;
    for (uint32_t w = 0; w < n_wheres; ++w) {
        std::vector<uint64_t> &terms = clauses[w].terms;
        terms.assign(where_terms + where_term_offsets[w], where_terms + where_term_offsets[w + 1]);
        std::sort(terms.begin(), terms.end());
        terms.erase(std::unique(terms.begin(), terms.end()), terms.end());
    }
    std::vector<uint32_t> canon(n_wheres);
    std::unordered_map<std::string, uint32_t> first_of;
    for (uint32_t w = 0; w < n_wheres; ++w) {
        const Clause &cl = clauses[w];
        canon[w] = w;
        if (cl.terms.empty()) continue;
        std::string key(reinterpret_cast<const char *>(&cl.pred), sizeof(WherePred));
        key.append(reinterpret_cast<const char *>(&cl.box), sizeof(LocBox));
        key.append(reinterpret_cast<const char *>(cl.terms.data()), cl.terms.size() * sizeof(uint64_t));
        canon[w] = first_of.emplace(std::move(key), w).first->second;
    }
    qw.resize(n_queries);
    for (uint32_t i = 0; i < n_queries; ++i) qw[i] = query_where[i] == WAX_VS_NO_FILTER ? WAX_VS_NO_FILTER : canon[query_where[i]];
    return WAX_VS_OK;
}

int32_t wax_vs_search_batch_where_terms(wax_vs_engine *e, const float *queries, uint32_t n_queries, uint32_t query_len,
                                        int64_t top_k, const uint64_t *frame_ids, const uint64_t *filter_offsets,
                                        const int32_t *filter_modes, uint32_t n_filters, const uint32_t *query_filter,
                                        const wax_vs_where_near *wheres, uint32_t n_wheres, const uint32_t *query_where,
                                        const uint64_t *where_term_offsets, const uint64_t *where_terms,
                                        uint64_t *out_ids, float *out_scores, uint32_t out_stride, uint32_t *out_n) {
    int32_t rc;
    if ((rc = check_where_args(e, n_queries, frame_ids, filter_offsets, filter_modes, n_filters, query_filter, wheres,
                               n_wheres, query_where, out_n)))
        return rc;
    if (!where_term_offsets) return fail(WAX_VS_ERR_NULL, "where_term_offsets is NULL");
    std::vector<Clause> clauses;
    std::vector<uint32_t> qw;
    if ((rc = term_clauses(wheres, n_wheres, query_where, n_queries, where_term_offsets, where_terms, clauses, qw)))
        return rc;
    return search_where_host(e, queries, n_queries, query_len, top_k, frame_ids, filter_offsets, filter_modes, n_filters,
                             query_filter, clauses, qw.data(), out_ids, out_scores, out_stride, out_n);
}

static int32_t reserve_shard_scratch(wax_vs_engine *e, SearchCtx *c) {
    const size_t rows = std::max<size_t>(e->n_rows, 1), words = (rows + 31) / 32;
    int32_t rc;
    if ((rc = c->d_queries.ensure(e->dims, "query buffer")) || (rc = c->h_queries.ensure(e->dims, "query staging")) ||
        (rc = c->d_out.ensure(kShardKCap, "result buffer")) || (rc = c->d_shard_local.ensure(kShardKCap, "shard candidates")) ||
        (rc = c->d_filter_rows.ensure(rows, "filter rows")) || (rc = c->d_mask.ensure(words, "row filters")) ||
        (rc = c->d_filter_spec.ensure(4, "filter spec")) || (rc = c->d_query_filter.ensure(1, "query filters")) ||
        (rc = c->d_gather_span.ensure(1, "gather spans")) || (rc = c->d_gather_keys.ensure(kWhereGatherRows, "gather keys")) ||
        (rc = c->d_where_items.ensure(1, "where predicates")) || (rc = c->d_where_counts.ensure(1, "where counts")) ||
        (rc = c->d_term_ids.ensure(kMaxWhereTerms, "required terms")) ||
        (rc = c->d_term_spans.ensure(kMaxWhereTerms, "term spans")) || (rc = c->d_term_units.ensure(1, "term units")) ||
        (rc = c->d_term_counts.ensure(1, "term counts")) || (rc = c->d_term_deny.ensure(rows, "term deny-lists")))
        return rc;
    return WAX_VS_OK;
}

static int32_t shard_search_host(wax_vs_engine *e, const float *query, uint32_t query_len, int64_t top_k, bool filtered,
                                 const uint64_t *frame_ids, uint64_t n_ids, int32_t mode, const Clause *where,
                                 uint64_t *out_ids, float *out_scores, uint32_t out_cap, uint32_t *out_n) {
    std::shared_lock<std::shared_mutex> r(e->rw);
    *out_n = 0;
    if (!e->shard.connected) return fail(WAX_VS_ERR_ARGUMENT, "the shard group is not connected (wax_vs_shard_open / _connect)");
    int32_t rc;
    if ((rc = check_query(e, query, query_len))) return rc;
    const uint32_t k_eff = clamp_topk(top_k);
    if (k_eff > static_cast<uint32_t>(kShardKCap))
        return fail(WAX_VS_ERR_UNSUPPORTED, "sharded search supports top_k <= %d (got %u)", kShardKCap, k_eff);
    if (!out_ids || !out_scores) return fail(WAX_VS_ERR_NULL, "output buffer is NULL");
    DeviceGuard g(e->device);
    if (!g.ok) return g.error();
    auto &sh = e->shard;
    std::lock_guard<std::mutex> sg(sh.mu);
    SearchCtx *c = sh.ctx;
    c->row_keys = device_row_keys(e);
    const uint64_t *d_ids = nullptr;
    if ((rc = sync_device_ids(e, &d_ids))) return rc;
    uint64_t launches = 0;
    const bool planned = filtered || where;
    const std::vector<Clause> wheres(where ? 1 : 0, where ? *where : Clause{});
    const uint32_t qw = where ? 0u : WAX_VS_NO_FILTER, qf = filtered && (mode == 0 || n_ids) ? 0u : WAX_VS_NO_FILTER;
    const uint64_t offsets[2] = {0, n_ids};
    FilterSet ids, fs;
    std::vector<int32_t> modes;
    std::vector<uint32_t> pair_of;
    FilteredPlan plan;
    if (planned && e->n_rows) {
        resolve_filters(e, frame_ids, offsets, 1, &qf, 1, ids);
        if ((rc = reserve_shard_scratch(e, c)) ||
            (rc = plan_where_pairs(e, c, wheres, &qw, &mode, &qf, 1, ids, fs, modes, pair_of)))
            return rc;
        plan_filtered(e, k_eff, modes.data(), pair_of.data(), 1, fs, plan);
    }
    ShardParams sp = shard_params_next(e);
    sp.host_out = sh.h_final; sp.host_flag = sh.h_flag;
    if (!planned) {
        HostDelivery hd{query, nullptr, nullptr, 0};
        rc = enqueue_search(e, c, nullptr, k_eff, sh.row_offset, sh.d_final, d_ids, c->stream, &launches, nullptr, &sp, &hd);
    } else if (plan.order.empty()) {
        sp.final_out = sh.d_final;
        if ((rc = c->d_shard_local.ensure(kShardKCap, "shard candidates"))) return rc;
        CUDA_TRY(cudaMemsetAsync(c->d_shard_local, 0, k_eff * sizeof(wax_vs_candidate), c->stream));
        rc = enqueue_exchange(sp, c->d_shard_local, k_eff, c->stream, &launches);
    } else {
        sp.final_out = sh.d_final;
        plan.k_max = plan.k_of[0] = k_eff;
        FilteredTarget tgt;
        tgt.row_offset = sh.row_offset; tgt.d_ids = d_ids; tgt.shard = &sp;
        rc = run_filtered(e, c, query, modes.data(), static_cast<uint32_t>(modes.size()), pair_of.data(), fs, plan, tgt);
    }
    if (rc) { cudaStreamSynchronize(c->stream); return rc; }
    if ((rc = shard_wait_host(e, sp.seq))) { cudaStreamSynchronize(c->stream); return rc; }
    if (planned) CUDA_TRY(cudaStreamSynchronize(c->stream));
    uint32_t m = 0;
    for (uint32_t i = 0; i < k_eff; ++i) {
        const wax_vs_candidate &cd = sh.h_final[i];
        if (cd.valid != 1u) continue;
        if (m >= out_cap) return fail(WAX_VS_ERR_BUFFER, "output buffers hold %u entries, need more", out_cap);
        out_ids[m] = cd.frame_id;
        out_scores[m] = score_from_distance(e->similarity, cd.distance);
        ++m;
    }
    *out_n = m;
    return WAX_VS_OK;
}

int32_t wax_vs_shard_search_where(wax_vs_engine *e, const float *query, uint32_t query_len, int64_t top_k,
                                  const uint64_t *frame_ids, uint64_t n_ids, int32_t mode, const wax_vs_where_near *where,
                                  const uint64_t *terms, uint32_t n_terms, uint64_t *out_ids, float *out_scores,
                                  uint32_t out_cap, uint32_t *out_n) {
    if (!e || !out_n || !where) return fail(WAX_VS_ERR_NULL, "NULL argument");
    if (mode != 0 && mode != 1) return fail(WAX_VS_ERR_ARGUMENT, "filter mode must be 0 (allow-list) or 1 (deny-list)");
    if (n_ids && !frame_ids) return fail(WAX_VS_ERR_NULL, "frame_ids is NULL");
    const uint64_t term_offsets[2] = {0, n_terms};
    std::vector<Clause> clauses;
    std::vector<uint32_t> qw;
    const uint32_t q0 = 0;
    int32_t rc;
    if ((rc = term_clauses(where, 1, &q0, 1, term_offsets, terms, clauses, qw))) return rc;
    return shard_search_host(e, query, query_len, top_k, true, frame_ids, n_ids, mode, &clauses[0], out_ids, out_scores,
                             out_cap, out_n);
}

int32_t wax_vs_search_batch_where_device(wax_vs_engine *e, const float *d_queries, uint32_t n_queries, int64_t top_k,
                                         const uint64_t *frame_ids, const uint64_t *filter_offsets,
                                         const int32_t *filter_modes, uint32_t n_filters, const uint32_t *query_filter,
                                         const wax_vs_where_near *wheres, uint32_t n_wheres, const uint32_t *query_where,
                                         const uint64_t *where_term_offsets, const uint64_t *where_terms,
                                         uint64_t row_offset, wax_vs_candidate *d_candidates, void *cuda_stream) {
    int32_t rc;
    uint32_t no_out_n = 0;
    if ((rc = check_where_args(e, n_queries, frame_ids, filter_offsets, filter_modes, n_filters, query_filter, wheres,
                               n_wheres, query_where, &no_out_n)))
        return rc;
    if (!d_queries || !d_candidates) return fail(WAX_VS_ERR_NULL, "NULL argument");
    std::vector<Clause> clauses;
    std::vector<uint32_t> qw;
    if (where_term_offsets) {
        rc = term_clauses(wheres, n_wheres, query_where, n_queries, where_term_offsets, where_terms, clauses, qw);
    } else {
        rc = near_clauses(wheres, n_wheres, clauses);
        qw.assign(query_where, query_where + n_queries);
    }
    if (rc) return rc;
    if (n_queries == 0) return WAX_VS_OK;
    std::shared_lock<std::shared_mutex> r(e->rw);
    DeviceGuard g(e->device);
    if (!g.ok) return g.error();
    SearchCtx *c = nullptr;
    if ((rc = ctx_for_stream(e, cuda_stream, &c))) return rc;
    const uint32_t k_out = clamp_topk(top_k);
    e->async_pending.store(true);
    CUDA_TRY(cudaMemsetAsync(d_candidates, 0, static_cast<size_t>(n_queries) * k_out * sizeof(wax_vs_candidate), c->stream));
    if (e->n_rows == 0) return WAX_VS_OK;
    const uint64_t *d_ids = nullptr;
    if ((rc = sync_device_ids(e, &d_ids))) return rc;
    FilterSet ids, fs;
    resolve_filters(e, frame_ids, filter_offsets, n_filters, query_filter, n_queries, ids);
    std::vector<int32_t> modes;
    std::vector<uint32_t> pair_of;
    if ((rc = plan_where_pairs(e, c, clauses, qw.data(), filter_modes, query_filter, n_queries, ids, fs, modes, pair_of)))
// ... 827 lines not shown
    const uint8_t magic[4] = {0x4D, 0x56, 0x32, 0x56};
    memcpy(p, magic, 4); p += 4;
    const uint16_t version = 1; memcpy(p, &version, 2); p += 2;
    *p++ = 2;
    *p++ = e->similarity;
    memcpy(p, &e->dims, 4); p += 4;
    memcpy(p, &e->n_rows, 8); p += 8;
    const uint64_t vbytes = e->n_rows * e->dims * 4ull;
    memcpy(p, &vbytes, 8); p += 8;
    memset(p, 0, 8); p += 8;
    if (vbytes) {
        std::lock_guard<std::mutex> ig(e->ingest_mu);
        int32_t rc = download_bytes(e, p, e->d_corpus, vbytes);
        if (rc) return rc;
    }
    p += vbytes;
    const uint64_t ibytes = e->n_rows * 8ull;
    memcpy(p, &ibytes, 8); p += 8;
    if (e->ids_identity) {
        for (uint64_t i = 0; i < e->n_rows; ++i) { const uint64_t id = e->id_base + i; memcpy(p + i * 8, &id, 8); }
    } else if (ibytes) {
        memcpy(p, e->ids.data(), ibytes);
    }
    return WAX_VS_OK;
}

static int32_t deserialize_rows(wax_vs_engine *e, const uint8_t *src, uint64_t len, bool all, uint64_t first, uint64_t n) {
    if (!e || !src) return fail(WAX_VS_ERR_NULL, "NULL argument");
    std::unique_lock<std::shared_mutex> w(e->rw);
    if (len < 36) return fail(WAX_VS_ERR_FORMAT, "Metal segment too small: %llu bytes", static_cast<unsigned long long>(len));
    const uint8_t magic[4] = {0x4D, 0x56, 0x32, 0x56};
    if (memcmp(src, magic, 4) != 0) return fail(WAX_VS_ERR_FORMAT, "Metal segment magic mismatch");
    uint16_t version; memcpy(&version, src + 4, 2);
    if (version != 1) return fail(WAX_VS_ERR_FORMAT, "Unsupported Metal segment version %u", version);
    if (src[6] != 2) return fail(WAX_VS_ERR_FORMAT, "Unsupported Metal segment encoding %u", src[6]);
    if (src[7] > 2 || src[7] != e->similarity)
        return fail(WAX_VS_ERR_FORMAT, "Metric mismatch: expected %u, got %u", e->similarity, src[7]);
    uint32_t dims; memcpy(&dims, src + 8, 4);
    if (dims != e->dims) return fail(WAX_VS_ERR_FORMAT, "Dimension mismatch: expected %u, got %u", e->dims, dims);
    uint64_t count, vbytes; memcpy(&count, src + 12, 8); memcpy(&vbytes, src + 20, 8);
    for (int i = 0; i < 8; ++i)
        if (src[28 + i] != 0) return fail(WAX_VS_ERR_FORMAT, "Metal segment reserved bytes must be zero");
    if (count > 0xFFFFFFFFull) return fail(WAX_VS_ERR_CAPACITY, "capacity exceeded: limit %llu, requested %llu", 0xFFFFFFFFull, static_cast<unsigned long long>(count));
    if (vbytes != count * static_cast<uint64_t>(dims) * 4ull) return fail(WAX_VS_ERR_FORMAT, "Vector data length mismatch");
    if (len < 36 + vbytes + 8) return fail(WAX_VS_ERR_FORMAT, "Metal segment missing frameId length");
    uint64_t ibytes; memcpy(&ibytes, src + 36 + vbytes, 8);
    if (ibytes != count * 8ull) return fail(WAX_VS_ERR_FORMAT, "FrameId data length mismatch");
    if (len != 36 + vbytes + 8 + ibytes)
        return fail(WAX_VS_ERR_FORMAT, "vec segment length mismatch: expected %llu, got %llu",
                    static_cast<unsigned long long>(36 + vbytes + 8 + ibytes), static_cast<unsigned long long>(len));
    if (all) first = 0, n = count;
    else if (first > count || n > count - first)
        return fail(WAX_VS_ERR_ARGUMENT, "rows [%llu, %llu + %llu) are outside the segment's %llu rows",
                    static_cast<unsigned long long>(first), static_cast<unsigned long long>(first),
                    static_cast<unsigned long long>(n), static_cast<unsigned long long>(count));
    const size_t row_bytes = static_cast<size_t>(dims) * 4u;
    DeviceGuard g(e->device);
    drain_device_path(e);
    int32_t rc = set_capacity(e, std::max<uint64_t>(n, 64));
    if (rc) return rc;
    if (n && (rc = upload_bytes(e, e->d_corpus, src + 36 + first * row_bytes, n * row_bytes)))
        return rc;
    e->n_rows = n;
    e->ids.resize(n);
    if (n) memcpy(e->ids.data(), src + 36 + vbytes + 8 + first * 8, n * 8);
    e->ids_identity = false;
    e->map_valid = false;
    e->ids_sorted = true;
    for (uint64_t i = 1; i < n && e->ids_sorted; ++i) e->ids_sorted = e->ids[i] > e->ids[i - 1];
    e->d_ids_dirty = true;
    e->keys_set = !all;
    e->keys.resize(e->keys_set ? n : 0);
    for (uint64_t i = 0; i < e->keys.size(); ++i) e->keys[i] = first + i;
    e->keys.shrink_to_fit();
    if ((rc = upload_row_keys(e, 0))) return rc;
    e->groups_set = false;
    e->groups.clear(); e->groups.shrink_to_fit();
    e->attrs_set = false;
    e->attrs.clear(); e->attrs.shrink_to_fit();
    e->locs_set = false;
    e->locs.clear(); e->locs.shrink_to_fit();
    clear_terms(e);
    invalidate_row_caches(e, 0);
    return WAX_VS_OK;
}

int32_t wax_vs_deserialize(wax_vs_engine *e, const uint8_t *src, uint64_t len) {
    return deserialize_rows(e, src, len, true, 0, 0);
}

int32_t wax_vs_deserialize_rows(wax_vs_engine *e, const uint8_t *src, uint64_t len, uint64_t first, uint64_t n) {
    return deserialize_rows(e, src, len, false, first, n);
}

int32_t wax_vs_export_rows(wax_vs_engine *e, uint64_t first, uint64_t n, uint64_t *out_ids, float *out_vectors,
                           uint64_t *out_keys) {
    if (!e) return fail(WAX_VS_ERR_NULL, "engine is NULL");
    std::shared_lock<std::shared_mutex> r(e->rw);
    if (first > e->n_rows || n > e->n_rows - first) return fail(WAX_VS_ERR_ARGUMENT, "row range out of bounds");
    for (uint64_t i = 0; i < n; ++i) {
        if (out_ids) out_ids[i] = frame_id_of(e, first + i);
        if (out_keys) out_keys[i] = e->keys_set ? e->keys[first + i] : first + i;
    }
    if (out_vectors && n) {
        DeviceGuard g(e->device);
        if (!g.ok) return g.error();
        std::lock_guard<std::mutex> ig(e->ingest_mu);
        return download_bytes(e, out_vectors, e->d_corpus + first * e->dims, n * e->dims * sizeof(float));
    }
    return WAX_VS_OK;
}

int32_t wax_vs_debug_pool_stats(wax_vs_engine *e, uint64_t *allocations, uint64_t *reuses) {
    if (!e) return fail(WAX_VS_ERR_NULL, "engine is NULL");
    std::lock_guard<std::mutex> g(e->pool_mu);
    if (allocations) *allocations = e->pool_allocs;
    if (reuses) *reuses = e->pool_reuses;
    return WAX_VS_OK;
}

int32_t wax_vs_debug_fill_synthetic(wax_vs_engine *e, uint64_t seed, uint64_t first_row, uint64_t rows,
                                    uint64_t id_base, int32_t normalize) {
    if (!e) return fail(WAX_VS_ERR_NULL, "engine is NULL");
    if (rows > 0xFFFFFFFFull) return fail(WAX_VS_ERR_CAPACITY, "capacity exceeded: limit %llu, requested %llu", 0xFFFFFFFFull, static_cast<unsigned long long>(rows));
    std::unique_lock<std::shared_mutex> w(e->rw);
    DeviceGuard g(e->device);
    drain_device_path(e);
    e->n_rows = 0;
    int32_t rc = set_capacity(e, std::max<uint64_t>(rows, 64));
    if (rc) return rc;
    if (rows) {
        const unsigned blocks = static_cast<unsigned>((rows + 255) / 256);
        synth_fill_kernel<<<blocks, 256>>>(e->d_corpus, rows, e->dims, seed, first_row, normalize);
        CUDA_TRY(cudaGetLastError());
        CUDA_TRY(cudaDeviceSynchronize());
    }
    e->n_rows = rows;
    e->ids.clear(); e->ids.shrink_to_fit();
    e->ids_identity = true; e->id_base = id_base;
    e->map = IdMap(); e->map_valid = true; e->ids_sorted = true;
    e->d_ids_dirty = true;
    e->keys_set = false;
    e->keys.clear(); e->keys.shrink_to_fit();
    e->groups_set = false;
    e->groups.clear(); e->groups.shrink_to_fit();
    e->attrs_set = false;
    e->attrs.clear(); e->attrs.shrink_to_fit();
    e->locs_set = false;
    e->locs.clear(); e->locs.shrink_to_fit();
    clear_terms(e);
    invalidate_row_caches(e, 0);
    return WAX_VS_OK;
}

int32_t wax_vs_debug_read_rows(wax_vs_engine *e, uint64_t first, uint64_t n, float *dst) {
    if (!e || !dst) return fail(WAX_VS_ERR_NULL, "NULL argument");
    std::shared_lock<std::shared_mutex> r(e->rw);
    if (first + n > e->n_rows) return fail(WAX_VS_ERR_ARGUMENT, "row range out of bounds");
    DeviceGuard g(e->device);
    if (n) CUDA_TRY(cudaMemcpy(dst, e->d_corpus + first * e->dims, n * e->dims * sizeof(float), cudaMemcpyDeviceToHost));
    return WAX_VS_OK;
}

int32_t wax_vs_debug_time_search(wax_vs_engine *e, uint32_t n_queries, int64_t top_k, uint64_t seed,
                                 uint32_t warmup, uint32_t iters, float *out_ms_total, uint64_t *out_launches) {
    if (!e || !out_ms_total) return fail(WAX_VS_ERR_NULL, "NULL argument");
    if (n_queries == 0) n_queries = 1;
    std::shared_lock<std::shared_mutex> r(e->rw);
    DeviceGuard g(e->device);
    CtxLease lease(e);
    int32_t rc = lease.acquire();
    if (rc) return rc;
    SearchCtx *c = lease.c;
    const uint32_t k_eff = clamp_topk(top_k);
    const size_t qfloats = static_cast<size_t>(n_queries) * e->dims;
    if ((rc = c->d_queries.ensure(qfloats, "query buffer"))) return rc;
    if ((rc = c->d_out.ensure(static_cast<size_t>(n_queries) * k_eff, "result buffer"))) return rc;
    synth_fill_kernel<<<(n_queries + 255) / 256, 256, 0, c->stream>>>(c->d_queries, n_queries, e->dims, seed, 0, 1);
    CUDA_TRY(cudaGetLastError());
    uint64_t launches = 0;
    CtxLease lease2(e);
    if (e->tune.time_overlap) {
        if ((rc = lease2.acquire())) return rc;
        if ((rc = lease2.c->d_out.ensure(static_cast<size_t>(n_queries) * k_eff, "result buffer"))) return rc;
    }
    SearchCtx *c2 = lease2.c;
    if (shadow_route_applies(e)) {
        bool use = false;
        RouteForm form = kRouteBf16;
        TmaConfig cfg{};
        if ((rc = select_route_form(e, c->stream, false, &use, &form, &cfg))) return rc;
    }
    for (uint32_t it = 0; it < warmup + iters; ++it) {
        if (it == warmup) {
            launches = 0;
            if (c2) { CUDA_TRY(cudaEventRecord(c2->ev0, c2->stream)); CUDA_TRY(cudaStreamWaitEvent(c->stream, c2->ev0, 0)); }
            CUDA_TRY(cudaEventRecord(c->ev0, c->stream));
            if (c2) CUDA_TRY(cudaStreamWaitEvent(c2->stream, c->ev0, 0));
        }
        const uint32_t qi = it % n_queries;
        SearchCtx *cc = (c2 && (it & 1u)) ? c2 : c;
        if (c2 && it == 0) { CUDA_TRY(cudaEventRecord(c->ev1, c->stream)); CUDA_TRY(cudaStreamWaitEvent(c2->stream, c->ev1, 0)); }
        rc = enqueue_search(e, cc, c->d_queries + static_cast<size_t>(qi) * e->dims, k_eff, 0,
                            cc->d_out + static_cast<size_t>(qi) * k_eff, nullptr, cc->stream, &launches, nullptr, nullptr,
                            nullptr, false, true);
        if (rc) { cudaStreamSynchronize(c->stream); if (c2) cudaStreamSynchronize(c2->stream); return rc; }
    }
    if (c2) { CUDA_TRY(cudaEventRecord(c2->ev1, c2->stream)); CUDA_TRY(cudaStreamWaitEvent(c->stream, c2->ev1, 0)); }
    CUDA_TRY(cudaEventRecord(c->ev1, c->stream));
    CUDA_TRY(cudaStreamSynchronize(c->stream));
    CUDA_TRY(cudaEventElapsedTime(out_ms_total, c->ev0, c->ev1));
    if (out_launches) *out_launches = launches;
    return WAX_VS_OK;
}

int32_t wax_vs_debug_stream_read(wax_vs_engine *e, uint32_t iters, float *out_best_ms, uint64_t *out_bytes) {
    if (!e || !out_best_ms || !out_bytes) return fail(WAX_VS_ERR_NULL, "NULL argument");
    std::shared_lock<std::shared_mutex> r(e->rw);
    DeviceGuard g(e->device);
    CtxLease lease(e);
    int32_t rc = lease.acquire();
    if (rc) return rc;
    SearchCtx *c = lease.c;
    const uint64_t bytes = e->n_rows * e->dims * sizeof(float) / 16 * 16;
    *out_bytes = bytes;
    *out_best_ms = 0.0f;
    if (bytes == 0) return WAX_VS_OK;
    float best = 1e30f;
    for (uint32_t it = 0; it < iters + 2; ++it) {
        CUDA_TRY(cudaEventRecord(c->ev0, c->stream));
        stream_read_kernel<<<e->sm_count * 4, 512, 0, c->stream>>>(reinterpret_cast<const uint4 *>(e->d_corpus),
                                                                     bytes / 16, c->d_ticket + 2);
        CUDA_TRY(cudaGetLastError());
        CUDA_TRY(cudaEventRecord(c->ev1, c->stream));
        CUDA_TRY(cudaStreamSynchronize(c->stream));
// ... 41 lines not shown
    if (!e || !out5) return fail(WAX_VS_ERR_NULL, "NULL argument");
    std::unique_lock<std::shared_mutex> w(e->rw);
    DeviceGuard g(e->device);
    CtxLease lease(e, true);
    int32_t rc = lease.acquire();
    if (rc) return rc;
    SearchCtx *c = lease.c;
    const uint32_t k_eff = clamp_topk(top_k);
    if ((rc = c->d_queries.ensure(static_cast<size_t>(e->dims), "query buffer"))) return rc;
    if ((rc = c->d_out.ensure(static_cast<size_t>(k_eff), "result buffer"))) return rc;
    synth_fill_kernel<<<1, 256, 0, c->stream>>>(c->d_queries, 1, e->dims, 99, 0, 1);
    unsigned long long *d_trace = nullptr;
    CUDA_TRY(cudaMalloc(&d_trace, 8 * sizeof(unsigned long long)));
    double acc[5] = {0, 0, 0, 0, 0};
    uint64_t launches = 0;
    for (uint32_t it = 0; it < iters + 3; ++it) {
        const unsigned long long init[8] = {~0ull, 0, 0, 0, 0, 0, 0, 0};
        cudaMemcpyAsync(d_trace, init, sizeof init, cudaMemcpyHostToDevice, c->stream);
        cudaStreamSynchronize(c->stream);
        e->debug_trace = d_trace;
        cudaEventRecord(c->ev0, c->stream);
        rc = enqueue_search(e, c, c->d_queries, k_eff, 0, c->d_out, nullptr, c->stream, &launches);
        cudaEventRecord(c->ev1, c->stream);
        e->debug_trace = nullptr;
        if (rc) { cudaStreamSynchronize(c->stream); cudaFree(d_trace); return rc; }
        unsigned long long t[8];
        cudaMemcpyAsync(t, d_trace, sizeof t, cudaMemcpyDeviceToHost, c->stream);
        cudaStreamSynchronize(c->stream);
        float ms = 0;
        cudaEventElapsedTime(&ms, c->ev0, c->ev1);
        if (it < 3) continue;
        for (int i = 0; i < 4; ++i) acc[i] += (t[i + 1] > t[0] && t[0] != ~0ull) ? (t[i + 1] - t[0]) * 1e-3 : 0.0;
        acc[4] += ms * 1e3;
    }
    cudaFree(d_trace);
    for (int i = 0; i < 5; ++i) out5[i] = static_cast<float>(acc[i] / std::max(iters, 1u));
    CUDA_TRY(cudaGetLastError());
    return WAX_VS_OK;
}

int32_t wax_vs_debug_batch_stats(wax_vs_engine *e, uint64_t *tensor_queries, uint64_t *fallback_queries) {
    if (!e) return fail(WAX_VS_ERR_NULL, "engine is NULL");
    std::lock_guard<std::mutex> g(e->pool_mu);
    if (tensor_queries) *tensor_queries = e->batch_tensor_queries;
    if (fallback_queries) *fallback_queries = e->batch_fallback_queries;
    return WAX_VS_OK;
}

int32_t wax_vs_debug_counter(wax_vs_engine *e, const char *name, uint64_t *out) {
    if (!e || !name || !out) return fail(WAX_VS_ERR_NULL, "NULL argument");
    std::lock_guard<std::mutex> g(e->pool_mu);
    const wax_vs_engine::Shadow &bf = e->shadows[kRouteBf16], &i8 = e->shadows[kRouteInt8], &u4 = e->shadows[kRouteU4];
    if (!strcmp(name, "batch_tensor_queries")) *out = e->batch_tensor_queries;
    else if (!strcmp(name, "batch_fallback_queries")) *out = e->batch_fallback_queries;
    else if (!strcmp(name, "batch_bf16_queries")) *out = e->batch_bf16_queries;
    else if (!strcmp(name, "batch_retry_queries")) *out = e->batch_retry_queries;
    else if (!strcmp(name, "batch_filter_bf16_queries")) *out = e->batch_filter_bf16_queries;
    else if (!strcmp(name, "shadow_bytes")) *out = bf.valid ? bf.rows * e->dims * sizeof(__nv_bfloat16) : 0;
    else if (!strcmp(name, "shadow_capacity_bytes")) *out = bf.codes.cap * sizeof(uint32_t);
    else if (!strcmp(name, "shadow_unavailable")) *out = bf.unavailable ? 1 : 0;
    else if (!strcmp(name, "batch_tf32_queries")) *out = e->batch_tf32_queries;
    else if (!strcmp(name, "filter_bitset_passes")) *out = e->filter_bitset_passes;
    else if (!strcmp(name, "group_index_builds")) *out = e->group_index_builds;
    else if (!strcmp(name, "attribute_uploads")) *out = e->attribute_uploads;
    else if (!strcmp(name, "location_uploads")) *out = e->location_uploads;
    else if (!strcmp(name, "term_index_builds")) *out = e->term_index_builds;
    else if (!strcmp(name, "term_index_bytes"))
        *out = e->tindex.keys.cap * sizeof(uint64_t) + e->tindex.start.cap * sizeof(uint64_t) + e->tindex.postings.cap * sizeof(uint32_t);
    else if (!strcmp(name, "grouped_batch_covered_queries")) *out = e->grouped_batch_covered_queries;
    else if (!strcmp(name, "grouped_batch_expanded_groups")) *out = e->grouped_batch_expanded_groups;
    else if (!strcmp(name, "grouped_batch_fallback_queries")) *out = e->grouped_batch_fallback_queries;
    else if (!strcmp(name, "grouped_batch_expansion_passes")) *out = e->grouped_batch_expansion_passes;
    else if (!strcmp(name, "shard_grouped_expanded_groups")) *out = e->shard_grouped_expanded_groups;
    else if (!strcmp(name, "ingest_h2d_bytes")) *out = e->ingest_h2d_bytes;
    else if (!strcmp(name, "ingest_d2h_bytes")) *out = e->ingest_d2h_bytes;
    else if (!strcmp(name, "norms_rows")) *out = e->norms_rows;
    else if (!strcmp(name, "shadow_rows")) *out = bf.rows;
    else if (!strcmp(name, "int8_shadow_bytes")) *out = i8.valid ? i8.rows * (e->dims + sizeof(float)) : 0;
    else if (!strcmp(name, "int8_shadow_rows")) *out = i8.rows;
    else if (!strcmp(name, "u4_shadow_bytes")) *out = u4.valid ? u4.rows * (e->dims / 2 + sizeof(float)) : 0;
    else if (!strcmp(name, "u4_shadow_rows")) *out = u4.rows;
    else if (!strcmp(name, "single_u4_queries")) *out = e->single_route_queries[kRouteU4];
    else if (!strcmp(name, "single_int8_queries")) *out = e->single_route_queries[kRouteInt8];
    else if (!strcmp(name, "batch_heap_bump")) *out = e->heap_bump;
    else if (!strcmp(name, "batch_last_heap")) *out = e->last_heap;
    else if (!strcmp(name, "single_shadow_queries") || !strcmp(name, "single_shadow_fallbacks")) {
        const int slot = !strcmp(name, "single_shadow_queries") ? 0 : 1;
        uint64_t n = 0;
        auto add = [&](const SearchCtx *c) { if (c->h_proof_count) n += *static_cast<volatile uint32_t *>(c->h_proof_count + slot); };
        for (const SearchCtx *c : e->pool) add(c);
        for (const auto &kv : e->stream_ctx) add(kv.second);
        *out = n;
    }
    else if (!strcmp(name, "pool_allocs")) *out = e->pool_allocs;
    else if (!strcmp(name, "pool_reuses")) *out = e->pool_reuses;
    else return fail(WAX_VS_ERR_ARGUMENT, "unknown counter '%s'", name);
    return WAX_VS_OK;
}

int32_t wax_vs_debug_time_search_batch(wax_vs_engine *e, uint32_t n_queries, int64_t top_k, uint64_t seed,
                                       uint32_t warmup, uint32_t iters, float *out_ms_total,
                                       uint64_t *out_launches, uint32_t *out_unproven) {
    if (!e || !out_ms_total) return fail(WAX_VS_ERR_NULL, "NULL argument");
    if (n_queries == 0) n_queries = 1;
    std::shared_lock<std::shared_mutex> r(e->rw);
    DeviceGuard g(e->device);
    const uint32_t k_eff = static_cast<uint32_t>(std::min<uint64_t>(clamp_topk(top_k), std::max<uint64_t>(e->n_rows, 1)));
    if (!batch_tensor_eligible(e, n_queries, k_eff))
        return fail(WAX_VS_ERR_UNSUPPORTED, "batch of %u queries, k=%u, dims=%u is not eligible for the tensor path", n_queries, k_eff, e->dims);
    CtxLease lease(e);
    int32_t rc = lease.acquire();
    if (rc) return rc;
    SearchCtx *c = lease.c;
    const size_t qfloats = static_cast<size_t>(n_queries) * e->dims;
    if ((rc = c->d_queries.ensure(qfloats, "query buffer"))) return rc;
    if ((rc = c->d_out.ensure(static_cast<size_t>(n_queries) * k_eff, "result buffer"))) return rc;
    if ((rc = c->d_ok.ensure(static_cast<size_t>(n_queries), "proof flags"))) return rc;
    if ((rc = c->h_ok.ensure(static_cast<size_t>(n_queries), "proof flag staging"))) return rc;
    synth_fill_kernel<<<(n_queries + 255) / 256, 256, 0, c->stream>>>(c->d_queries, n_queries, e->dims, seed, 0, 1);
    CUDA_TRY(cudaGetLastError());
    if ((rc = ensure_norms(e, c->stream))) return rc;
    if (batch_bf16_wanted(e) && (rc = ensure_shadow(e, c->stream))) return rc;
    uint64_t launches = 0;
    for (uint32_t it = 0; it < warmup + iters; ++it) {
        if (it == warmup) { launches = 0; CUDA_TRY(cudaEventRecord(c->ev0, c->stream)); }
        uint32_t used_heap = 0;
        rc = enqueue_batch_tensor(e, c, c->d_queries, n_queries, k_eff, 0, c->d_out, c->d_ok, nullptr, c->stream, &launches,
                                  true, nullptr, nullptr, RowFilter{}, &used_heap);
        if (rc) { cudaStreamSynchronize(c->stream); return rc; }
        if (used_heap) { std::lock_guard<std::mutex> pg(e->pool_mu); e->last_heap = used_heap; }
    }
    CUDA_TRY(cudaEventRecord(c->ev1, c->stream));
    CUDA_TRY(cudaMemcpyAsync(c->h_ok, c->d_ok, n_queries * sizeof(uint32_t), cudaMemcpyDeviceToHost, c->stream));
    CUDA_TRY(cudaStreamSynchronize(c->stream));
    CUDA_TRY(cudaEventElapsedTime(out_ms_total, c->ev0, c->ev1));
    if (out_launches) *out_launches = launches;
    if (out_unproven) {
        uint32_t bad = 0;
        for (uint32_t i = 0; i < n_queries; ++i) bad += c->h_ok[i] ? 0u : 1u;
        *out_unproven = bad;
    }
    return WAX_VS_OK;
}

int32_t wax_vs_debug_batch_nominations(wax_vs_engine *e, const float *queries, uint32_t n_queries, int64_t top_k,
                                       const uint32_t *allow_bits, float *out_scores, uint32_t *out_ok,
                                       uint64_t *out_heaps, uint64_t heaps_cap, uint32_t *out_shape) {
    if (!e || !queries || !out_scores || !out_ok || !out_shape) return fail(WAX_VS_ERR_NULL, "NULL argument");
    std::shared_lock<std::shared_mutex> r(e->rw);
    DeviceGuard g(e->device);
    if (!g.ok) return g.error();
    const uint32_t k_eff = static_cast<uint32_t>(std::min<uint64_t>(clamp_topk(top_k), std::max<uint64_t>(e->n_rows, 1)));
    if (n_queries == 0 || e->n_rows == 0 || k_eff > 128u || e->dims % kBatchKBlock != 0 || e->dims > 8192 ||
        (e->similarity != WAX_VS_COSINE && e->similarity != WAX_VS_DOT && !(e->similarity == WAX_VS_L2 && e->tune.batch_l2)))
        return fail(WAX_VS_ERR_UNSUPPORTED, "batch of %u queries, k=%u, dims=%u has no tensor-core nomination pass",
                    n_queries, k_eff, e->dims);
    CtxLease lease(e);
    int32_t rc = lease.acquire();
    if (rc) return rc;
    SearchCtx *c = lease.c;
    const size_t qfloats = static_cast<size_t>(n_queries) * e->dims;
    const size_t n_scores = static_cast<size_t>(n_queries) * e->n_rows;
    if ((rc = c->d_queries.ensure(qfloats, "query buffer"))) return rc;
    if ((rc = c->d_out.ensure(static_cast<size_t>(n_queries) * k_eff, "result buffer"))) return rc;
    if ((rc = c->d_ok.ensure(static_cast<size_t>(n_queries), "proof flags"))) return rc;
    DevBuf<float> scores;
    if ((rc = scores.ensure(n_scores, "nomination scores"))) return rc;
    CUDA_TRY(cudaMemsetAsync(scores, 0xFF, n_scores * sizeof(float), c->stream));
    CUDA_TRY(cudaMemcpyAsync(c->d_queries, queries, qfloats * sizeof(float), cudaMemcpyHostToDevice, c->stream));
    const uint32_t *d_mask = nullptr;
    if (allow_bits) {
        const size_t words = static_cast<size_t>((e->n_rows + 31) / 32);
        if ((rc = c->d_mask.ensure(words, "row filter"))) return rc;
        CUDA_TRY(cudaMemcpyAsync(c->d_mask, allow_bits, words * sizeof(uint32_t), cudaMemcpyHostToDevice, c->stream));
// ... 94 lines not shown
                                    uint32_t *out_shape, float *out_bound) {
    return debug_route_nominations(e, query, top_k, allow_bits, out_keys, out_ok, out_result, out_shape, kRouteU4,
                                   keys_cap, out_bound);
}

static int32_t debug_read_route_shadow(wax_vs_engine *e, RouteForm f, uint64_t first, uint64_t n, void *dst_codes,
                                       float *dst_scales, float *out_rho_max) {
    const RouteFormSpec &fs = kRouteSpec[f];
    std::shared_lock<std::shared_mutex> r(e->rw);
    if (first > e->n_rows || n > e->n_rows - first) return fail(WAX_VS_ERR_ARGUMENT, "row range out of bounds");
    TmaConfig cfg{};
    if (f == kRouteBf16 ? !batch_bf16_wanted(e)
                        : (e->similarity != WAX_VS_COSINE && e->similarity != WAX_VS_DOT) || !pick_route_config(e, f, &cfg))
        return fail(WAX_VS_ERR_UNSUPPORTED, "no %s shadow for dims=%u with this metric and these options", fs.name, e->dims);
    DeviceGuard g(e->device);
    if (!g.ok) return g.error();
    CtxLease lease(e);
    int32_t rc = lease.acquire();
    if (rc) return rc;
    if ((rc = ensure_route_shadow(e, f, lease.c->stream, true))) return rc;
    const wax_vs_engine::Shadow &sh = e->shadows[f];
    if (!sh.valid) return fail(WAX_VS_ERR_UNSUPPORTED, "the %s shadow does not fit in device memory", fs.name);
    const size_t words = shadow_words(e, f);
    if (n) {
        CUDA_TRY(cudaMemcpy(dst_codes, sh.codes + first * words, n * words * sizeof(uint32_t), cudaMemcpyDeviceToHost));
        if (fs.scaled) CUDA_TRY(cudaMemcpy(dst_scales, sh.scale + first, n * sizeof(float), cudaMemcpyDeviceToHost));
    }
    if (fs.scaled) *out_rho_max = sh.rho_max;
    return WAX_VS_OK;
}

int32_t wax_vs_debug_read_u4_shadow(wax_vs_engine *e, uint64_t first, uint64_t n, uint8_t *dst_codes, float *dst_half_steps,
                                    float *out_rho_max) {
    if (!e || !dst_codes || !dst_half_steps || !out_rho_max) return fail(WAX_VS_ERR_NULL, "NULL argument");
    return debug_read_route_shadow(e, kRouteU4, first, n, dst_codes, dst_half_steps, out_rho_max);
}

int32_t wax_vs_debug_read_int8_shadow(wax_vs_engine *e, uint64_t first, uint64_t n, uint8_t *dst_codes, float *dst_scales,
                                      float *out_rho_max) {
    if (!e || !dst_codes || !dst_scales || !out_rho_max) return fail(WAX_VS_ERR_NULL, "NULL argument");
    return debug_read_route_shadow(e, kRouteInt8, first, n, dst_codes, dst_scales, out_rho_max);
}

int32_t wax_vs_debug_read_shadow(wax_vs_engine *e, uint64_t first, uint64_t n, uint16_t *dst) {
    if (!e || !dst) return fail(WAX_VS_ERR_NULL, "NULL argument");
    return debug_read_route_shadow(e, kRouteBf16, first, n, dst, nullptr, nullptr);
}

int32_t wax_vs_debug_set_option(wax_vs_engine *e, const char *key, int64_t value) {
    if (!e || !key) return fail(WAX_VS_ERR_NULL, "NULL argument");
    std::unique_lock<std::shared_mutex> w(e->rw);
    const int v = static_cast<int>(value);
    if (!strcmp(key, "variant")) e->tune.variant = v;
    else if (!strcmp(key, "rows_per_step")) e->tune.rows_per_step = v;
    else if (!strcmp(key, "stages")) e->tune.stages = v;
    else if (!strcmp(key, "warps")) e->tune.warps = v;
    else if (!strcmp(key, "grid")) e->tune.grid = v;
    else if (!strcmp(key, "l2_hint")) e->tune.l2_hint = v;
    else if (!strcmp(key, "chunk_steps")) e->tune.chunk_steps = v;
    else if (!strcmp(key, "fused_k_max")) e->tune.fused_k_max = std::max(0, std::min(128, v));
    else if (!strcmp(key, "batch_tensor")) e->tune.batch_tensor = v;
    else if (!strcmp(key, "batch_min")) e->tune.batch_min = v;
    else if (!strcmp(key, "batch_noinsert")) e->tune.batch_noinsert = v;
    else if (!strcmp(key, "batch_heap")) e->tune.batch_heap = v;
    else if (!strcmp(key, "batch_large_k")) e->tune.batch_large_k = v;
    else if (!strcmp(key, "tma_max_dims")) e->tune.tma_max_dims = static_cast<uint32_t>(std::max(v, 0));
    else if (!strcmp(key, "batch_pair")) e->tune.batch_pair = v;
    else if (!strcmp(key, "batch_ares")) e->tune.batch_ares = v;
    else if (!strcmp(key, "batch_bf16")) { e->tune.batch_bf16 = v; e->shadows[kRouteBf16].unavailable = false; e->bf16_skip_batches = 0; }
    else if (!strcmp(key, "batch_rescore")) e->tune.batch_rescore = v;
    else if (!strcmp(key, "batch_retry")) e->tune.batch_retry = v;
    else if (!strcmp(key, "filter_cap")) e->tune.filter_cap = v;
    else if (!strcmp(key, "filter_bf16")) e->tune.filter_bf16 = v;
    else if (!strcmp(key, "batch_l2")) e->tune.batch_l2 = v;
    else if (!strcmp(key, "filter_bitset_bytes")) e->tune.filter_bitset_bytes = static_cast<uint64_t>(std::max<int64_t>(value, 0));
    else if (!strcmp(key, "single_shadow")) e->tune.single_shadow = v;
    else if (!strcmp(key, "shadow_scan")) {
        std::lock_guard<std::mutex> pg(e->pool_mu);
        e->tune.shadow_scan = v;
        e->shadow_scan_skip = 0;
        auto seen = [](SearchCtx *c) { if (c->h_proof_count) c->seen_failed = *static_cast<volatile uint32_t *>(c->h_proof_count + 1); };
        for (SearchCtx *c : e->pool) seen(c);
        for (auto &kv : e->stream_ctx) seen(kv.second);
    }
    else if (!strcmp(key, "shadow_rows_per_step")) e->tune.route[kRouteBf16].rows_per_step = v;
    else if (!strcmp(key, "shadow_warps")) e->tune.route[kRouteBf16].warps = v;
    else if (!strcmp(key, "shadow_stages")) e->tune.route[kRouteBf16].stages = v;
    else if (!strcmp(key, "shadow_scan_min_bytes")) e->tune.route[kRouteBf16].min_bytes = static_cast<uint64_t>(std::max<int64_t>(value, 0));
    else if (!strcmp(key, "int8_scan_min_bytes")) {
        e->tune.route[kRouteInt8].min_bytes = static_cast<uint64_t>(std::max<int64_t>(value, 0));
        e->shadows[kRouteInt8].unavailable = false;
        e->shadows[kRouteInt8].coarse = false;
    }
    else if (!strcmp(key, "u4_scan_min_bytes")) {
        e->tune.route[kRouteU4].min_bytes = static_cast<uint64_t>(std::max<int64_t>(value, 0));
        e->shadows[kRouteU4].unavailable = false;
        e->shadows[kRouteU4].coarse = false;
        e->u4_demoted = 0; e->u4_demote_window = 16; e->u4_probing = false;
    }
    else if (!strcmp(key, "u4_rows_per_step")) e->tune.route[kRouteU4].rows_per_step = v;
    else if (!strcmp(key, "u4_warps")) e->tune.route[kRouteU4].warps = v;
    else if (!strcmp(key, "u4_stages")) e->tune.route[kRouteU4].stages = v;
    else if (!strcmp(key, "int8_rows_per_step")) e->tune.route[kRouteInt8].rows_per_step = v;
    else if (!strcmp(key, "int8_warps")) e->tune.route[kRouteInt8].warps = v;
    else if (!strcmp(key, "int8_stages")) e->tune.route[kRouteInt8].stages = v;
    else if (!strcmp(key, "shard_fused")) e->tune.shard_fused = v;
    else if (!strcmp(key, "tail_select")) e->tune.tail_select = v;
    else if (!strcmp(key, "inline_query")) e->tune.inline_query = v;
    else if (!strcmp(key, "host_delivery")) e->tune.host_delivery = v;
    else if (!strcmp(key, "shard_timeout_ms")) e->shard.timeout_ns = static_cast<unsigned long long>(std::max<int64_t>(value, 1)) * 1000000ull;
    else if (!strcmp(key, "time_overlap")) e->tune.time_overlap = v;
    else if (!strcmp(key, "ldg_ctas_per_sm")) e->tune.ldg_ctas_per_sm = std::max(1, v);
    else return fail(WAX_VS_ERR_ARGUMENT, "unknown option '%s'", key);
    return WAX_VS_OK;
}

}
```

wax_b200/csrc/waxvs_scan.cuh:

```cuda
#pragma once
#include "waxvs_common.cuh"
#include "waxvs_shard.cuh"
#include "../../include/wax_vs_cuda.h"

namespace waxvs {

constexpr int kInlineQueryFloats = 512;

struct ScanParams {
    const float *corpus;
    const float *query;
    uint32_t n_rows;
    uint32_t dims;
    uint32_t k;
    uint32_t stages;
    uint64_t *block_keys;
    uint32_t *ticket;
    wax_vs_candidate *out;
    uint32_t *dist_keys;
    const uint64_t *frame_ids;
    uint64_t id_base;
    uint64_t row_offset;
    const uint64_t *row_keys;
    uint32_t use_l2_hint;
// ... 220 lines not shown
        if (tk.key[j] != WAXVS_KEY_NONE && tk.key[j] <= xa) mine[atomicAdd(&ss.n_sel, 1u)] = tk.key[j];
    __syncthreads();
    for (uint32_t i = ss.n_sel + tid; i < k; i += nthr) mine[i] = WAXVS_KEY_NONE;
    __threadfence();
    __syncthreads();
    if (p.trace && tid == 0) atomicMax(p.trace + 2, global_timer_ns());
    if (tid == 0) s_last2 = (atomicAdd(p.ticket, 1u) == gridDim.x - 1) ? 1u : 0u;
    __syncthreads();
    if (!s_last2) return false;
    __threadfence();
    if (p.trace && tid == 0) p.trace[3] = global_timer_ns();
    const uint32_t total = gridDim.x * k;
    const bool staged = static_cast<size_t>(total) * sizeof(uint64_t) <= p.tail_smem_bytes;
    uint64_t *sk = reinterpret_cast<uint64_t *>(scratch);
    if (staged) {
        for (uint32_t i = tid; i < total; i += nthr) sk[i] = ld_cg_u64(p.block_keys + i);
        __syncthreads();
    }
    auto grid_keys = [&](auto f) {
        if (staged) { for (uint32_t i = tid; i < total; i += nthr) f(sk[i]); }
        else { for (uint32_t i = tid; i < total; i += nthr) f(ld_cg_u64(p.block_keys + i)); }
    };
    const uint64_t xb = block_select_kth(grid_keys, k, &ss);
    if (tid == 0) ss.n_sel = 0;
    __syncthreads();
    grid_keys([&](uint64_t key) { if (key != WAXVS_KEY_NONE && key <= xb) ss.sel[atomicAdd(&ss.n_sel, 1u)] = key; });
    __syncthreads();
    const uint32_t n_sel = ss.n_sel;
    for (uint32_t i = tid; i < k; i += nthr) {
        if (i < n_sel) {
            const uint64_t key = ss.sel[i];
            uint32_t rank = 0;
            for (uint32_t j = 0; j < n_sel; ++j) rank += ss.sel[j] < key ? 1u : 0u;
            write_slot<SHADOW>(p, static_cast<int>(rank), key);
        } else {
            write_slot<SHADOW>(p, static_cast<int>(i), WAXVS_KEY_NONE);
        }
    }
    if (p.host_flag && !p.shard.world) __threadfence_system();
    __syncthreads();
    if (tid == 0) {
        *p.ticket = 0u;
        if (p.work_counter) *p.work_counter = 0u;
        if (p.host_flag && !p.shard.world) st_release_sys_u64(p.host_flag, p.host_seq);
        if (p.trace) p.trace[4] = global_timer_ns();
    }
    if (p.shard.world) shard_exchange_cta(p.shard, p.out, p.k, reinterpret_cast<uint32_t *>(scratch));
    return true;
}

template <int E>
__device__ __forceinline__ void finish_u4_nominees(const ScanParams &p, WarpTopK<E> &tk) {
    __shared__ SelectScratch ss;
    __shared__ uint32_t s_cut;
    const uint32_t tid = threadIdx.x, nthr = blockDim.x;
    if (tid == 0) s_cut = WAXVS_UKEY_NONE;
    auto own_keys = [&](auto f) {
#pragma unroll
        for (int j = 0; j < E; ++j) f(tk.key[j]);
    };
    const uint64_t xa = nthr * E >= kU4CtaNominees ? block_select_kth(own_keys, kU4CtaNominees, &ss) : WAXVS_KEY_NONE;
    if (tid == 0) ss.n_sel = 0;
    __syncthreads();
    uint64_t *mine = p.nominees + static_cast<size_t>(blockIdx.x) * kU4CtaNominees;
#pragma unroll
    for (int j = 0; j < E; ++j)
        if (tk.key[j] != WAXVS_KEY_NONE && tk.key[j] <= xa) mine[atomicAdd(&ss.n_sel, 1u)] = tk.key[j];
    if ((tid & 31u) == 0 && tk.thresh != WAXVS_KEY_NONE) atomicMin(&s_cut, static_cast<uint32_t>(tk.thresh >> 32));
    __syncthreads();
    for (uint32_t i = ss.n_sel + tid; i < kU4CtaNominees; i += nthr) mine[i] = WAXVS_KEY_NONE;
    if (tid == 0) {
        uint32_t cut = s_cut;
        if (xa != WAXVS_KEY_NONE) cut = min(cut, static_cast<uint32_t>(xa >> 32));
        if (cut != WAXVS_UKEY_NONE) atomicMin(p.u4_aux, cut);
    }
}

template <int C, int R, int METRIC, int E, bool EMIT, bool SHADOW = false, bool INT8 = false, bool U4 = false>
__global__ void __launch_bounds__(512, 1) scan_tma_kernel(const __grid_constant__ ScanParams p) {
    static_assert(!SHADOW || (C > 0 && METRIC != kL2 && !EMIT), "the shadow form covers the unrolled cosine / dot shapes");
    static_assert(!INT8 || (SHADOW && R >= 4), "the int8 form is a shadow form with 16-byte scale copies");
    static_assert(!U4 || (SHADOW && !INT8 && R >= 4 && E == 4), "the 4-bit form is a shadow form with 16-byte scale copies");
    constexpr bool SCALED = INT8 || U4;
    if constexpr (!SHADOW && !EMIT && E == 1 && METRIC != kL2) {
        if (p.proof_ok) {
            const bool proven = *p.proof_ok != 0u;
            if (blockIdx.x == 0) {
                if (threadIdx.x == 0) {
                    const uint32_t n = ++p.proof_count[proven ? 0 : 1];
                    *static_cast<volatile uint32_t *>(p.proof_count_host + (proven ? 0 : 1)) = n;
                }
                if (proven && p.host_flag) {
                    for (uint32_t i = threadIdx.x; i < p.k; i += blockDim.x) p.host_out[i] = p.out[i];
                    __threadfence_system();
                    __syncthreads();
                    if (threadIdx.x == 0) st_release_sys_u64(p.host_flag, p.host_seq);
                }
            }
            if (proven) return;
        }
    }
    const int D4 = C > 0 ? 32 * C : static_cast<int>(p.dims / 4u);
    const int CN = C > 0 ? C : (D4 + 31) / 32;
    const uint32_t ROW_BYTES = C > 0 ? (U4 ? 64u : INT8 ? 128u : SHADOW ? 256u : 512u) * C : p.dims * 4u;
    const uint32_t STAGE_BYTES = ROW_BYTES * R + (SCALED ? R * 4u : 0u);
    constexpr int LANES_PER_ROW = 32 / R;

    extern __shared__ __align__(128) unsigned char smem[];
    const int warp = threadIdx.x >> 5, lane = threadIdx.x & 31, warps = blockDim.x >> 5;
    const uint32_t stages = p.stages;
    unsigned char *ring = smem + static_cast<size_t>(warp) * stages * STAGE_BYTES;
    uint64_t *bars = reinterpret_cast<uint64_t *>(smem + static_cast<size_t>(warps) * stages * STAGE_BYTES) +
                     warp * stages;
    uint64_t *lists = reinterpret_cast<uint64_t *>(smem + static_cast<size_t>(warps) * stages * STAGE_BYTES) +
                      warps * stages;
    uint32_t *stage_step = reinterpret_cast<uint32_t *>(lists + warps * 32 * E) + warp * stages;
    float4 *qs = reinterpret_cast<float4 *>(reinterpret_cast<uint32_t *>(lists + warps * 32 * E) + warps * stages + 4);

    float4 q[C > 0 ? C : 1];
    const float4 *q4 = reinterpret_cast<const float4 *>(p.query);
    const float4 *qp = reinterpret_cast<const float4 *>(p.query_inline);
    auto load_q = [&](int i) -> float4 { return q4 ? __ldg(q4 + i) : qp[i]; };
    if (C > 0) {
#pragma unroll
        for (int c = 0; c < (C > 0 ? C : 1); ++c) q[c] = load_q(lane + 32 * c);
    } else {
        qs = reinterpret_cast<float4 *>((reinterpret_cast<uintptr_t>(qs) + 15) & ~uintptr_t(15));
        for (int i = threadIdx.x; i < CN * 32; i += blockDim.x) qs[i] = (i < D4) ? load_q(i) : make_float4(0.f, 0.f, 0.f, 0.f);
        __syncthreads();
    }
    auto qchunk = [&](int c) -> float4 { return C > 0 ? q[C > 0 ? c : 0] : qs[lane + 32 * c]; };
    if constexpr (SHADOW) {
        if (p.query_store && p.query == nullptr && blockIdx.x == 0)
            for (uint32_t i = threadIdx.x; i < p.dims; i += blockDim.x) p.query_store[i] = p.query_inline[i];
    }
    constexpr int CU = U4 ? (C > 0 ? C : 1) : 1;
    constexpr int H = U4 ? R / 2 : 1;
    const int hl = lane & 15, hh = lane >> 4;
    int qlo[CU], qhi[CU], word_of[CU];
    int q_code_sum = 0;
    float s_q = 0.0f;
    if constexpr (U4) {
        float m = 0.0f;
        bool bad = false;
#pragma unroll
        for (int c = 0; c < CU; ++c) {
            bad |= !finite_f32(q[c].x) || !finite_f32(q[c].y) || !finite_f32(q[c].z) || !finite_f32(q[c].w);
            m = fmaxf(m, fmaxf(fmaxf(fabsf(q[c].x), fabsf(q[c].y)), fmaxf(fabsf(q[c].z), fabsf(q[c].w))));
        }
#pragma unroll
        for (int o = 16; o > 0; o >>= 1) m = fmaxf(m, __shfl_xor_sync(WAXVS_FULL_MASK, m, o));
        bad = __any_sync(WAXVS_FULL_MASK, bad);
        s_q = __fdiv_rn(m, 127.0f);
        const bool code_it = !bad && s_q > 0.0f && finite_f32(s_q);
        double r2 = 0.0;
#pragma unroll
        for (int c = 0; c < CU; ++c) {
            word_of[c] = hl + 16 * ((C % 2 == 0) ? (c ^ hh) : c);
            int packed[2];
#pragma unroll
            for (int half = 0; half < 2; ++half) {
                const float4 x4 = load_q(2 * word_of[c] + half);
                const float xs[4] = {x4.x, x4.y, x4.z, x4.w};
                uint32_t w = 0;
#pragma unroll
                for (int j = 0; j < 4; ++j) {
                    const int code = code_it ? max(-127, min(127, __float2int_rn(__fdiv_rn(xs[j], s_q)))) : 0;
                    w |= static_cast<uint32_t>(code & 0xFF) << (8 * j);
                    const double e = static_cast<double>(xs[j]) - static_cast<double>(s_q) * static_cast<double>(code);
                    r2 = fma(e, e, r2);
                }
                packed[half] = static_cast<int>(w);
                q_code_sum = __dp4a(packed[half], 0x01010101, q_code_sum);
            }
            qlo[c] = packed[0]; qhi[c] = packed[1];
        }
#pragma unroll
        for (int o = 8; o > 0; o >>= 1) {
            q_code_sum += __shfl_xor_sync(WAXVS_FULL_MASK, q_code_sum, o);
            r2 += __shfl_xor_sync(WAXVS_FULL_MASK, r2, o);
        }
        if (blockIdx.x == 0 && threadIdx.x == 0) {
            float rho_q = __double2float_ru(sqrt(r2) * (1.0 + 0x1p-40));
            if (bad || !finite_f32(s_q) || !finite_f32(rho_q)) rho_q = INFINITY;
            p.u4_aux[1] = __float_as_uint(rho_q);
        }
    }
    float a2 = 0.0f, sqrt_a2 = 0.0f;
    if (METRIC == kCosine && !SHADOW) {
        float s0 = 0.f, s1 = 0.f, s2 = 0.f, s3 = 0.f;
#pragma unroll
// ... 298 lines not shown
```

Baseline: 1442.

## Enable shadow route for sharded search and overlap fallback scan via dependent launch

Lets the compressed shadow route run for sharded searches above a size threshold. The proven-result exchange is performed inside the early-exit fallback scan kernel. The fallback scan is now launched with programmatic stream serialization, and the rescore kernel triggers dependents early, so launch latency between them overlaps. Route scratch buffers and kernel modules are reserved and loaded ahead of time on data changes rather than on first query. This adds host-side preparation work on every mutation and relies on griddepcontrol ordering for correctness.

```diff
diff --git a/wax_b200/csrc/waxvs_batch.cuh b/wax_b200/csrc/waxvs_batch.cuh
--- a/wax_b200/csrc/waxvs_batch.cuh
+++ b/wax_b200/csrc/waxvs_batch.cuh
@@ -969,6 +969,7 @@
 template <int METRIC>
 __global__ void __launch_bounds__(512, 1) shadow_rescore_kernel(const RescoreParams p) {
     static_assert(METRIC == kCosine || METRIC == kDot, "the shadow route covers cosine and dot");
+    grid_dependents_launch();
     extern __shared__ __align__(16) unsigned char rsm[];
     __shared__ float s_a2, s_sqrt_a2;
     const int warp = threadIdx.x >> 5, lane = threadIdx.x & 31, warps = blockDim.x >> 5;
diff --git a/wax_b200/csrc/waxvs_common.cuh b/wax_b200/csrc/waxvs_common.cuh
--- a/wax_b200/csrc/waxvs_common.cuh
+++ b/wax_b200/csrc/waxvs_common.cuh
@@ -275,6 +275,9 @@
     asm volatile("createpolicy.fractional.L2::evict_first.b64 %0, 1.0;" : "=l"(pol));
     return pol;
 }
+__device__ __forceinline__ void grid_dependency_wait() { asm volatile("griddepcontrol.wait;" ::: "memory"); }
+__device__ __forceinline__ void grid_dependents_launch() { asm volatile("griddepcontrol.launch_dependents;" ::: "memory"); }
+
 __device__ __forceinline__ uint64_t ld_cg_u64(const uint64_t *p) {
     uint64_t v;
     asm volatile("ld.global.cg.u64 %0, [%1];" : "=l"(v) : "l"(p) : "memory");
diff --git a/wax_b200/csrc/waxvs_engine.cu b/wax_b200/csrc/waxvs_engine.cu
--- a/wax_b200/csrc/waxvs_engine.cu
+++ b/wax_b200/csrc/waxvs_engine.cu
@@ -166,6 +166,8 @@
     int host_delivery = 1;
     int tail_select = 1;
     int shard_fused = 1;
+    int shard_route = 1;
+    uint64_t shard_route_min_bytes = 1638ull << 20;
     int batch_l2 = 0;
     int single_shadow = 0;
     uint64_t filter_bitset_bytes = 2ull << 30;
@@ -304,6 +306,7 @@
     uint32_t u4_demoted = 0, u4_demote_window = 16;
     bool u4_probing = false;
     uint64_t single_route_queries[kRouteForms] = {};
+    uint64_t shard_route_collective_allocs = 0;
     uint64_t batch_tensor_queries = 0, batch_fallback_queries = 0;
     uint64_t batch_bf16_queries = 0, batch_retry_queries = 0, batch_tf32_queries = 0, batch_filter_bf16_queries = 0;
     uint64_t filter_bitset_passes = 0;
@@ -500,6 +503,7 @@
     }
     int32_t acquire() { return ctx_acquire(e, &c); }
 };
+static int32_t reserve_route_scratch(wax_vs_engine *e, SearchCtx *c, cudaStream_t stream);
 static int32_t ctx_for_stream(wax_vs_engine *e, void *cuda_stream, SearchCtx **out) {
     std::lock_guard<std::mutex> pg(e->pool_mu);
     auto it = e->stream_ctx.find(cuda_stream);
@@ -513,6 +517,7 @@
     if (rc) return rc;
     c->stream = static_cast<cudaStream_t>(cuda_stream);
     c->row_keys = device_row_keys(e);
+    if (e->shard.open && (rc = reserve_route_scratch(e, c, c->stream))) { delete c; return rc; }
     e->stream_ctx[cuda_stream] = c;
     ++e->pool_allocs;
     *out = c;
@@ -582,10 +587,30 @@
     return err;
 }
 
+template <typename K>
+static cudaError_t load_kernel(K kernel) {
+    cudaFuncAttributes a;
+    return cudaFuncGetAttributes(&a, kernel);
+}
+
+template <typename K, typename P>
+static cudaError_t launch_dependent(K kernel, int grid, int threads, size_t smem, cudaStream_t s, const P &params) {
+    cudaLaunchConfig_t cfg{};
+    cfg.gridDim = dim3(grid); cfg.blockDim = dim3(threads); cfg.dynamicSmemBytes = smem; cfg.stream = s;
+    cudaLaunchAttribute attr[1];
+    attr[0].id = cudaLaunchAttributeProgrammaticStreamSerialization;
+    attr[0].val.programmaticStreamSerializationAllowed = 1;
+    cfg.attrs = attr; cfg.numAttrs = 1;
+    return cudaLaunchKernelEx(&cfg, kernel, params);
+}
+
 template <int C, int R, int M, int E, bool EMIT, bool SHADOW = false, bool INT8 = false, bool U4 = false>
 static cudaError_t launch_tma_inst(wax_vs_engine *e, const ScanParams &p, int grid, const TmaConfig &cfg, cudaStream_t s) {
     cudaError_t err = grant_smem(e, scan_tma_kernel<C, R, M, E, EMIT, SHADOW, INT8, U4>, cfg.smem);
     if (err != cudaSuccess) return err;
+    if (grid == 0) return load_kernel(scan_tma_kernel<C, R, M, E, EMIT, SHADOW, INT8, U4>);
+    if (p.proof_ok) return launch_dependent(scan_tma_kernel<C, R, M, E, EMIT, SHADOW, INT8, U4>, grid, cfg.warps * 32,
+                                            cfg.smem, s, p);
     scan_tma_kernel<C, R, M, E, EMIT, SHADOW, INT8, U4><<<grid, cfg.warps * 32, cfg.smem, s>>>(p);
     return cudaGetLastError();
 }
@@ -806,13 +831,39 @@
         if ((f == kRouteU4 && demoted) || e->n_rows * e->dims * sizeof(float) < e->tune.route[f].min_bytes ||
             !pick_route_config(e, f, cfg))
             continue;
-        if (const int32_t rc = ensure_route_shadow(e, f, stream)) return rc;
-        if (e->shadows[f].valid && e->shadows[f].eps_rel <= kRouteSpec[f].max_eps_rel) {
+        if (!e->shard.connected)
+            if (const int32_t rc = ensure_route_shadow(e, f, stream)) return rc;
+        if (e->shadows[f].valid && e->shadows[f].rows == e->n_rows && e->shadows[f].eps_rel <= kRouteSpec[f].max_eps_rel) {
             *use = true;
             *form = f;
             return WAX_VS_OK;
         }
     }
+    return WAX_VS_OK;
+}
+
+static size_t route_nominee_keys(const wax_vs_engine *e) {
+    return std::max(static_cast<size_t>(kShadowNominees) * kNomineeStride,
+                    static_cast<size_t>(std::max(e->tune.grid, e->sm_count)) * kU4CtaNominees);
+}
+static bool route_scratch_ready(const wax_vs_engine *e, const SearchCtx *c) {
+    return c->h_proof_count && c->d_u4_aux && c->d_ok && c->d_heaps.cap >= route_nominee_keys(e) && c->d_queries.cap >= e->dims;
+}
+static int32_t reserve_route_scratch(wax_vs_engine *e, SearchCtx *c, cudaStream_t stream) {
+    int32_t rc;
+    if (!c->h_proof_count) {
+        if ((rc = c->d_proof_count.ensure(2, "proof counts")) || (rc = c->h_proof_count.ensure(2, "proof count mirror"))) return rc;
+        CUDA_TRY(cudaMemsetAsync(c->d_proof_count, 0, 2 * sizeof(uint32_t), stream));
+        c->h_proof_count[0] = c->h_proof_count[1] = 0;
+        c->seen_failed = 0;
+    }
+    if (!c->d_u4_aux) {
+        if ((rc = c->d_u4_aux.ensure(3, "4-bit route state"))) return rc;
+        CUDA_TRY(cudaMemsetAsync(c->d_u4_aux, 0xFF, 3 * sizeof(uint32_t), stream));
+    }
+    if ((rc = c->d_heaps.ensure(route_nominee_keys(e), "nominee keys")) || (rc = c->d_ok.ensure(1, "proof flags")) ||
+        (rc = c->d_queries.ensure(e->dims, "query buffer")))
+        return rc;
     return WAX_VS_OK;
 }
 
@@ -820,15 +871,7 @@
                                           cudaStream_t stream, uint64_t *launches, uint32_t *shape, RouteForm f) {
     const RouteFormSpec &fs = kRouteSpec[f];
     const wax_vs_engine::Shadow &sh = e->shadows[f];
-    int32_t rc;
-    if (fs.grid_rescore && !c->d_u4_aux) {
-        if ((rc = c->d_u4_aux.ensure(3, "4-bit route state"))) return rc;
-        CUDA_TRY(cudaMemsetAsync(c->d_u4_aux, 0xFF, 3 * sizeof(uint32_t), stream));
-    }
-    const size_t cta_keys = static_cast<size_t>(std::max(e->tune.grid, e->sm_count)) * kU4CtaNominees;
-    if ((rc = c->d_heaps.ensure(std::max(static_cast<size_t>(kShadowNominees) * kNomineeStride, fs.grid_rescore ? cta_keys : 0), "nominee keys")) ||
-        (rc = c->d_ok.ensure(1, "proof flags")) || (!p.query && (rc = c->d_queries.ensure(e->dims, "query buffer"))))
-        return rc;
+    if (const int32_t rc = reserve_route_scratch(e, c, stream)) return rc;
 
     ScanParams sp = p;
     sp.corpus = reinterpret_cast<const float *>(sh.codes.p);
@@ -836,6 +879,7 @@
     sp.u4_aux = fs.grid_rescore ? c->d_u4_aux.p : nullptr;
     sp.k = kShadowNominees;
     sp.out = nullptr; sp.host_out = nullptr; sp.host_flag = nullptr;
+    sp.shard = ShardParams{};
     sp.nominees = c->d_heaps;
     sp.query_store = p.query ? nullptr : c->d_queries.p;
     sp.tail_select = e->tune.tail_select ? 1u : 0u;
@@ -879,14 +923,16 @@
     return WAX_VS_OK;
 }
 
-static int32_t enqueue_shadow_route(wax_vs_engine *e, SearchCtx *c, ScanParams &p, cudaStream_t stream, uint64_t *launches) {
+static int32_t enqueue_shadow_route(wax_vs_engine *e, SearchCtx *c, ScanParams &p, cudaStream_t stream, uint64_t *launches,
+                                    bool collective) {
     if (!shadow_route_applies(e)) return WAX_VS_OK;
     int32_t rc;
-    if (!c->h_proof_count) {
-        if ((rc = c->d_proof_count.ensure(2, "proof counts")) || (rc = c->h_proof_count.ensure(2, "proof count mirror"))) return rc;
-        CUDA_TRY(cudaMemsetAsync(c->d_proof_count, 0, 2 * sizeof(uint32_t), stream));
-        c->h_proof_count[0] = c->h_proof_count[1] = 0;
-        c->seen_failed = 0;
+    if (!route_scratch_ready(e, c)) {
+        if (collective) {
+            std::lock_guard<std::mutex> pg(e->pool_mu);
+            ++e->shard_route_collective_allocs;
+        }
+        if ((rc = reserve_route_scratch(e, c, stream))) return rc;
     }
     bool demoted;
     {
@@ -925,6 +971,40 @@
     return WAX_VS_OK;
 }
 
+static int32_t sync_device_ids(wax_vs_engine *e, const uint64_t **out);
+static int32_t prepare_shard_route(wax_vs_engine *e) {
+    if (!e->shard.open) return WAX_VS_OK;
+    SearchCtx *sc = e->shard.ctx;
+    const uint64_t *d_ids = nullptr;
+    int32_t rc = sync_device_ids(e, &d_ids);
+    if (rc) return rc;
+    {
+        std::lock_guard<std::mutex> pg(e->pool_mu);
+        if ((rc = reserve_route_scratch(e, sc, sc->stream))) return rc;
+        for (auto &kv : e->stream_ctx)
+            if ((rc = reserve_route_scratch(e, kv.second, sc->stream))) return rc;
+    }
+    if (e->n_rows && shadow_route_applies(e) && e->n_rows * e->dims * sizeof(float) >= e->tune.shard_route_min_bytes) {
+        TmaConfig cfg{};
+        const ScanParams none{};
+        for (const RouteForm f : {kRouteU4, kRouteInt8, kRouteBf16}) {
+            if (e->n_rows * e->dims * sizeof(float) < e->tune.route[f].min_bytes || !pick_route_config(e, f, &cfg)) continue;
+            if ((rc = ensure_route_shadow(e, f, sc->stream))) return rc;
+            const bool usable = e->shadows[f].valid && e->shadows[f].eps_rel <= kRouteSpec[f].max_eps_rel;
+            if (usable) CUDA_TRY(kRouteSpec[f].launch(e, &none, 0, cfg, e->similarity, nullptr));
+            if (f != kRouteU4 && usable) break;
+        }
+        const bool cos = e->similarity == WAX_VS_COSINE;
+        TmaConfig fcfg{};
+        if (pick_tma_config(e, &fcfg, 0)) CUDA_TRY(launch_tma(e, none, 0, fcfg, e->similarity, 0, nullptr));
+        CUDA_TRY(cos ? load_kernel(batch_finish_kernel<kCosine>) : load_kernel(batch_finish_kernel<kDot>));
+        CUDA_TRY(cos ? load_kernel(shadow_rescore_kernel<kCosine>) : load_kernel(shadow_rescore_kernel<kDot>));
+        CUDA_TRY(load_kernel(shard_exchange_kernel));
+    }
+    CUDA_TRY(cudaStreamSynchronize(sc->stream));
+    return WAX_VS_OK;
+}
+
 static ScanParams scan_params(const wax_vs_engine *e, SearchCtx *c, const float *d_query, uint32_t k_eff, uint64_t row_offset,
                               wax_vs_candidate *d_out, const uint64_t *d_ids, const uint32_t *d_mask) {
     ScanParams p{};
@@ -1016,8 +1096,9 @@
         fused_exchange = e->tune.shard_fused != 0 && static_cast<size_t>(shard->world) * k_eff * sizeof(uint32_t) <= list_bytes;
         if (fused_exchange) { p.shard = *shard; p.shard.final_out = d_merged; }
     }
-    if (shadow_route && !shard && mode == 0 && use_tma && cfg.C > 0) {
-        int32_t rc = enqueue_shadow_route(e, c, p, stream, launches);
+    if (shadow_route && mode == 0 && use_tma && cfg.C > 0 &&
+        (!shard || (e->tune.shard_route && e->n_rows * e->dims * sizeof(float) >= e->tune.shard_route_min_bytes))) {
+        int32_t rc = enqueue_shadow_route(e, c, p, stream, launches, shard != nullptr);
         if (rc) return rc;
     }
     int grid;
@@ -1901,7 +1982,7 @@
         invalidate_row_caches(e, n0);
         rc = upload_bytes(e, e->d_corpus + n0 * e->dims, rows, n * row_bytes);
         tr.mark("upload");
-        return rc;
+        return rc ? rc : prepare_shard_route(e);
     }
     invalidate_row_caches(e, 0);
     {
@@ -1923,7 +2004,7 @@
         CUDA_TRY(cudaGetLastError());
         CUDA_TRY(cudaStreamSynchronize(ig.stream));
     }
-    return WAX_VS_OK;
+    return prepare_shard_route(e);
 }
 
 int32_t wax_vs_add_batch(wax_vs_engine *e, const uint64_t *frame_ids, const float *rows, uint64_t n,
@@ -2035,7 +2116,7 @@
     if ((rc = upload_row_keys(e, first))) return rc;
     tr.mark("compact ids");
     if (out_removed) *out_removed = gone.size();
-    return WAX_VS_OK;
+    return prepare_shard_route(e);
 }
 
 int32_t wax_vs_remove(wax_vs_engine *e, uint64_t frame_id) {
@@ -2478,7 +2559,7 @@
     h.magic = 0x48535857u; h.version = 1; h.pid = static_cast<int32_t>(getpid()); h.device = e->device;
     h.nonce = process_nonce(); h.ptr = reinterpret_cast<uint64_t>(box); h.rank = rank; h.world = world;
     memcpy(out_handle, &h, sizeof h);
-    return WAX_VS_OK;
+    return prepare_shard_route(e);
 }
 
 int32_t wax_vs_shard_connect(wax_vs_engine *e, const uint8_t *handles, int32_t n_handles) {
@@ -2561,7 +2642,7 @@
     ShardParams sp = shard_params_next(e);
     uint64_t launches = 0;
     return enqueue_search(e, c, d_query, k_eff, e->shard.row_offset, d_candidates, d_ids,
-                          static_cast<cudaStream_t>(cuda_stream), &launches, nullptr, &sp);
+                          static_cast<cudaStream_t>(cuda_stream), &launches, nullptr, &sp, nullptr, false, true);
 }
 
 static int32_t shard_wait_host(wax_vs_engine *e, unsigned long long seq) {
@@ -2605,7 +2686,7 @@
         if (it == warmup) { launches = 0; CUDA_TRY(cudaEventRecord(c->ev0, c->stream)); }
         ShardParams sp = shard_params_next(e);
         rc = enqueue_search(e, c, c->d_queries + static_cast<size_t>(it % n_queries) * e->dims, k_eff, sh.row_offset,
-                            sh.d_final, d_ids, c->stream, &launches, nullptr, &sp);
+                            sh.d_final, d_ids, c->stream, &launches, nullptr, &sp, nullptr, false, true);
         if (rc) { cudaStreamSynchronize(c->stream); return rc; }
     }
     CUDA_TRY(cudaEventRecord(c->ev1, c->stream));
@@ -3622,7 +3703,7 @@
         (rc = c->d_term_spans.ensure(kMaxWhereTerms, "term spans")) || (rc = c->d_term_units.ensure(1, "term units")) ||
         (rc = c->d_term_counts.ensure(1, "term counts")) || (rc = c->d_term_deny.ensure(rows, "term deny-lists")))
         return rc;
-    return WAX_VS_OK;
+    return reserve_route_scratch(e, c, c->stream);
 }
 
 static int32_t shard_search_host(wax_vs_engine *e, const float *query, uint32_t query_len, int64_t top_k, bool filtered,
@@ -3665,7 +3746,8 @@
     sp.host_out = sh.h_final; sp.host_flag = sh.h_flag;
     if (!planned) {
         HostDelivery hd{query, nullptr, nullptr, 0};
-        rc = enqueue_search(e, c, nullptr, k_eff, sh.row_offset, sh.d_final, d_ids, c->stream, &launches, nullptr, &sp, &hd);
+        rc = enqueue_search(e, c, nullptr, k_eff, sh.row_offset, sh.d_final, d_ids, c->stream, &launches, nullptr, &sp, &hd,
+                            false, true);
     } else if (plan.order.empty()) {
         sp.final_out = sh.d_final;
         if ((rc = c->d_shard_local.ensure(kShardKCap, "shard candidates"))) return rc;
@@ -4659,7 +4741,7 @@
     e->locs.clear(); e->locs.shrink_to_fit();
     clear_terms(e);
     invalidate_row_caches(e, 0);
-    return WAX_VS_OK;
+    return prepare_shard_route(e);
 }
 
 int32_t wax_vs_deserialize(wax_vs_engine *e, const uint8_t *src, uint64_t len) {
@@ -4727,7 +4809,7 @@
     e->locs.clear(); e->locs.shrink_to_fit();
     clear_terms(e);
     invalidate_row_caches(e, 0);
-    return WAX_VS_OK;
+    return prepare_shard_route(e);
 }
 
 int32_t wax_vs_debug_read_rows(wax_vs_engine *e, uint64_t first, uint64_t n, float *dst) {
@@ -4935,6 +5017,8 @@
     else if (!strcmp(name, "u4_shadow_rows")) *out = u4.rows;
     else if (!strcmp(name, "single_u4_queries")) *out = e->single_route_queries[kRouteU4];
     else if (!strcmp(name, "single_int8_queries")) *out = e->single_route_queries[kRouteInt8];
+    else if (!strcmp(name, "single_bf16_queries")) *out = e->single_route_queries[kRouteBf16];
+    else if (!strcmp(name, "shard_route_collective_allocs")) *out = e->shard_route_collective_allocs;
     else if (!strcmp(name, "batch_heap_bump")) *out = e->heap_bump;
     else if (!strcmp(name, "batch_last_heap")) *out = e->last_heap;
     else if (!strcmp(name, "single_shadow_queries") || !strcmp(name, "single_shadow_fallbacks")) {
@@ -4943,6 +5027,7 @@
         auto add = [&](const SearchCtx *c) { if (c->h_proof_count) n += *static_cast<volatile uint32_t *>(c->h_proof_count + slot); };
         for (const SearchCtx *c : e->pool) add(c);
         for (const auto &kv : e->stream_ctx) add(kv.second);
+        if (e->shard.ctx) add(e->shard.ctx);
         *out = n;
     }
     else if (!strcmp(name, "pool_allocs")) *out = e->pool_allocs;
@@ -5203,6 +5288,7 @@
         auto seen = [](SearchCtx *c) { if (c->h_proof_count) c->seen_failed = *static_cast<volatile uint32_t *>(c->h_proof_count + 1); };
         for (SearchCtx *c : e->pool) seen(c);
         for (auto &kv : e->stream_ctx) seen(kv.second);
+        if (e->shard.ctx) seen(e->shard.ctx);
     }
     else if (!strcmp(key, "shadow_rows_per_step")) e->tune.route[kRouteBf16].rows_per_step = v;
     else if (!strcmp(key, "shadow_warps")) e->tune.route[kRouteBf16].warps = v;
@@ -5226,6 +5312,8 @@
     else if (!strcmp(key, "int8_warps")) e->tune.route[kRouteInt8].warps = v;
     else if (!strcmp(key, "int8_stages")) e->tune.route[kRouteInt8].stages = v;
     else if (!strcmp(key, "shard_fused")) e->tune.shard_fused = v;
+    else if (!strcmp(key, "shard_route")) e->tune.shard_route = v;
+    else if (!strcmp(key, "shard_route_min_bytes")) e->tune.shard_route_min_bytes = static_cast<uint64_t>(std::max<int64_t>(value, 0));
     else if (!strcmp(key, "tail_select")) e->tune.tail_select = v;
     else if (!strcmp(key, "inline_query")) e->tune.inline_query = v;
     else if (!strcmp(key, "host_delivery")) e->tune.host_delivery = v;
diff --git a/wax_b200/csrc/waxvs_scan.cuh b/wax_b200/csrc/waxvs_scan.cuh
--- a/wax_b200/csrc/waxvs_scan.cuh
+++ b/wax_b200/csrc/waxvs_scan.cuh
@@ -326,8 +326,10 @@
     static_assert(!INT8 || (SHADOW && R >= 4), "the int8 form is a shadow form with 16-byte scale copies");
     static_assert(!U4 || (SHADOW && !INT8 && R >= 4 && E == 4), "the 4-bit form is a shadow form with 16-byte scale copies");
     constexpr bool SCALED = INT8 || U4;
+    extern __shared__ __align__(128) unsigned char smem[];
     if constexpr (!SHADOW && !EMIT && E == 1 && METRIC != kL2) {
         if (p.proof_ok) {
+            grid_dependency_wait();
             const bool proven = *p.proof_ok != 0u;
             if (blockIdx.x == 0) {
                 if (threadIdx.x == 0) {
@@ -340,6 +342,7 @@
                     __syncthreads();
                     if (threadIdx.x == 0) st_release_sys_u64(p.host_flag, p.host_seq);
                 }
+                if (proven && p.shard.world) shard_exchange_cta(p.shard, p.out, p.k, reinterpret_cast<uint32_t *>(smem));
             }
             if (proven) return;
         }
@@ -350,7 +353,6 @@
     const uint32_t STAGE_BYTES = ROW_BYTES * R + (SCALED ? R * 4u : 0u);
     constexpr int LANES_PER_ROW = 32 / R;
 
-    extern __shared__ __align__(128) unsigned char smem[];
     const int warp = threadIdx.x >> 5, lane = threadIdx.x & 31, warps = blockDim.x >> 5;
     const uint32_t stages = p.stages;
     unsigned char *ring = smem + static_cast<size_t>(warp) * stages * STAGE_BYTES;
```

New measurement: 1446 (median of 6 runs). Within noise of the previous version (+0.2%).
